# jsourati/nn-active-learning

Hardware: AMD Instinct MI355X
Metric: patches/sec Fisher-scored (32^3, 2-class) (higher is better)
Workload: dtype f32 (fp32 operands split into 16-bit pieces on the 16-bit MFMA, fp32 accumulate: fp16 pairs - 22-23 bits kept per operand, three products - in the conv under the head (forward + backward), in dec1's forward launch and in the other backward launches; bf16 triples - all 24 bits, exact, six products -

## Files before the change

### include/alq.h

```cpp
#ifndef ALQ_H
#define ALQ_H

#include <stddef.h>
#include <stdint.h>

#ifdef __cplusplus
extern "C" {
#endif

typedef struct alq_ctx alq_ctx;
typedef struct alq_model alq_model;

enum { ALQ_OK = 0, ALQ_EINVAL = -1, ALQ_EHIP = -2, ALQ_ENOMEM = -3, ALQ_EUNSUPPORTED = -4 };

enum { ALQ_CONV = 0, ALQ_CONVT = 1, ALQ_POOL = 2, ALQ_FC = 3 };

typedef struct {
    int32_t type;
    int32_t cout;
    int32_t k[3];
    int32_t s[3];
    int32_t relu;
    int32_t skip_src;
} alq_layer_t;
// ... 58 lines not shown

int alq_fisher_rows(alq_model *m, const float *d_pool, const int64_t *d_rows, int N, const float *d_p1_in,
                    double diag_load, float *d_p1_out, double *d_g0, double *d_g1, double *d_A,
                    double *d_trace, double *d_Asum);

int64_t alq_model_num_params(const alq_model *m);

int alq_forward_dropout(alq_model *m, const float *d_x, int N, float keep_prob, uint64_t seed, int64_t first_sample,
                        const int32_t *h_drop_layers, int n_drop_layers, float *d_post, int64_t *d_pred);

int alq_param_grads(alq_model *m, const float *d_x, int N, int mode, int cls, const int32_t *d_labels,
                    float loss_scale, float keep_prob, uint64_t seed, int64_t first_sample,
                    const int32_t *h_drop_layers, int n_drop_layers, int per_sample, float *d_grads,
                    float *d_post, double *d_loss);

int alq_grad_sqnorms(alq_model *m, const float *d_x, int N, int cls, const int32_t *d_cls,
                     float *d_post, double *d_sq);

int alq_hess_vecp(alq_model *m, const float *d_x, int N, const int32_t *d_labels, float loss_scale, const float *d_v,
                  const uint8_t *h_layer_on, int accumulate, double *d_hv, double *d_loss);

int alq_sgd_step(alq_ctx *ctx, float *d_theta, const float *d_grad, int64_t n, float lr);
int alq_adam_step(alq_ctx *ctx, float *d_theta, const float *d_grad, float *d_m, float *d_v, int64_t n, float lr,
                  float beta1, float beta2, float eps, int64_t t);
enum { ALQ_LOSS_CE = 0, ALQ_LOSS_CE_SOFT = 1, ALQ_LOSS_GCE = 2 };
typedef struct alq_loss_t {
    int32_t kind;
    float focal_gamma;
    float gce_q;
    float lwf_T;
    const float *d_class_w;
    const float *d_sample_w;
    const float *d_targets;
    const float *d_old_logits;
} alq_loss_t;

int alq_loss_stats(alq_ctx *ctx, const float *d_post, int c, int N, const int32_t *d_labels, const alq_loss_t *loss,
                   double *d_stats3);

int alq_param_grads_loss(alq_model *m, const float *d_x, int N, const int32_t *d_labels, const alq_loss_t *loss,
                         float loss_scale, float lwf_scale, float keep_prob, uint64_t seed, int64_t first_sample,
                         const int32_t *h_drop_layers, int n_drop_layers, float *d_grads, float *d_post, double *d_stats3);

int alq_rmsprop_step(alq_ctx *ctx, float *d_theta, const float *d_grad, float *d_ms, float *d_mom, int64_t n, float lr,
                     float decay, float momentum, float eps);

int alq_sq_accum(alq_ctx *ctx, const float *d_grads, int64_t per_sample_len, int N, double *d_acc);

int alq_shrink_sum(alq_ctx *ctx, const float *d_grads, int N, int64_t P, const int64_t *h_layer_elems, int L, double *d_out);
int alq_class_layer_sums(alq_model *m, const float *d_x, int N, int J, const int32_t *d_cls, float *d_post, double *d_g);

int alq_diag_fisher(alq_model *m, const float *d_x, int N, const int32_t *d_cls, double *d_acc);

size_t alq_topk_mask_work_bytes(int64_t n);
int alq_topk_mask(alq_ctx *ctx, const double *d_v, int64_t n, int64_t k, float *d_mask, void *d_work);
int alq_threshold_mask(alq_ctx *ctx, const double *d_v, int64_t n, double thr, float *d_mask);
int alq_fisher_classes(alq_ctx *ctx, const double *d_g, const double *d_w, const double *d_diag, int N, int c, int L,
                       double *d_A);

int alq_row_norms(alq_ctx *ctx, const float *d_A, int64_t n, int f, double *d_norms);
int alq_cosine_sims(alq_ctx *ctx, const float *d_A, int64_t n, const float *d_B, int b, int f, const double *d_na,
                    const double *d_nb, double *d_C);
size_t alq_colsum_work_bytes(int64_t n, int b);
int alq_colsum_max(alq_ctx *ctx, const double *d_S, int64_t n, int b, const double *d_cmax,
                   const unsigned char *d_skip, double *d_out, void *d_work);
int alq_take_colmax(alq_ctx *ctx, const double *d_S, int64_t n, int b, int j, int first, double *d_v);
int alq_fold_rowmax(alq_ctx *ctx, const double *d_S, int t, int64_t n, double *d_v);

int alq_local_var2d(alq_ctx *ctx, const void *d_vol, int vol_is_f64, const int64_t pad_dims[3], const int32_t rads[3], int d,
                    const int64_t *d_inds, int64_t n, double *d_out);
int alq_segment_min(alq_ctx *ctx, const int32_t *d_labels, const int64_t dims[3], int32_t n_labels, const int64_t *d_inds,
                    const double *d_scores, int64_t n, double *d_table);

size_t alq_cc_work_bytes(const int64_t dims[3]);
int alq_cc_label(alq_ctx *ctx, const uint8_t *d_seg, const int64_t dims[3], int connectivity, int select_zero, int32_t *d_labels);
int alq_cc_keep_largest(alq_ctx *ctx, const uint8_t *d_seg, const int64_t dims[3], int connectivity, int skip_origin, uint8_t *d_out,
                        int64_t *d_info, void *d_work);
int alq_fill_holes(alq_ctx *ctx, const uint8_t *d_seg, const int64_t dims[3], uint8_t *d_out, int64_t *d_info, void *d_work);

typedef struct alq_dcrf_params {
    float sdims_smooth[2];
    float sdims_app[2];
    float schan;
    float compat_smooth, compat_app;
    int32_t niter;
} alq_dcrf_params;
size_t alq_dcrf_work_bytes(const int64_t dims[3]);
int alq_dcrf2d(alq_ctx *ctx, const float *d_post, const float *d_img, const int64_t dims[3], const alq_dcrf_params *par,
               float *d_q1, uint8_t *d_map, void *d_work);

int alq_llfc_grads(alq_ctx *ctx, const float *d_feat, const float *d_post, const int32_t *d_labels, int n, int d, int c,
                   float *d_out);
size_t alq_llfc_hess_max_bytes(void);
int alq_llfc_hess(alq_ctx *ctx, const float *d_feat_one, const float *d_post_one, int d, int c, double *d_H);
int alq_llfc_if_path(int d, int c);
size_t alq_llfc_if_work_bytes(int n_pool, int c);
int alq_llfc_stoch_if(alq_ctx *ctx, const float *d_pool_feat, const float *d_pool_post, const int32_t *d_pool_labels, int n_pool,
                      const float *d_tr_feat, const float *d_tr_post, int n_tr, const int32_t *d_draws, int T, double scale, int d,
                      int c, int path, float *d_V, void *d_work);

int alq_aopt_tile(void);
int alq_aopt_max_workgroups(void);
size_t alq_aopt_work_bytes(int64_t n, int L);
int alq_aopt_svec(alq_ctx *ctx, const double *d_A, int64_t n, int L, double *d_V);
int alq_aopt_stats(alq_ctx *ctx, const double *d_V, const double *d_q, int64_t n, int m, const double *h_kvec,
                   const double *h_R, double mu, double obj, double *d_out, void *d_work);
int alq_aopt_direction(alq_ctx *ctx, const double *d_V, const double *d_q, int64_t n, int m, const double *h_kvec,
                       const double *h_R, const double *h_c_r, const double *h_c_1, double ratio, double mu, double obj,
                       double *d_dq, double *d_out, void *d_work);
int alq_aopt_linesearch(alq_ctx *ctx, const double *d_q, const double *d_dq, int64_t n, const double *h_alpha, int J,
                        double *d_out, void *d_work);
int alq_aopt_update(alq_ctx *ctx, double *d_q, const double *d_dq, const double *d_V, int64_t n, int m, double alpha,
                    double *d_out, void *d_work);

typedef struct {
    int32_t layer;
    int32_t pad;
    int64_t idx;
    double delta;
} alq_flip_t;
int alq_ref64_scores(alq_ctx *ctx, const alq_layer_t *layers, int n_layers, const int32_t in_dims[4],
                     const double *const *h_dW, const double *const *h_db, const float *d_x, const int64_t *d_rows, int N,
                     const alq_flip_t *d_flips, int flips_per_sample, double eps, int cand_cap,
                     double *d_logits, double *d_S, double *d_rms, alq_flip_t *d_cand, double *d_cand_key, int32_t *d_cand_count);

int alq_prof_enable(alq_ctx *ctx, int on);
int alq_prof_reset(alq_ctx *ctx);
int alq_prof_num_classes(void);
const char *alq_prof_class_name(int cls);
int alq_prof_read(alq_ctx *ctx, int cls, double *ms, int64_t *launches, double *flops);

int alq_model_debug_copy(alq_model *m, int layer_idx, int what, int N, float *d_out,
                         int64_t *elems_out);

int alq_debug_set_stamp_buffer(void *d_buf);
int alq_debug_set(int key, int value);
enum {
    ALQ_INFO_SUBNORMALS_OK = 0,
    ALQ_INFO_C3D_FWD = 1,
    ALQ_INFO_C3D_BWD = 2,
    ALQ_INFO_C3D_ONE_ACC = 3,
    ALQ_INFO_FLIP_OVERFLOW = 5,
    ALQ_INFO_F16_DERIVED = 6,
    ALQ_INFO_T3D_FWD = 7,
    ALQ_INFO_T3D_BWD = 8,
    ALQ_INFO_E3D_BWD = 9,
    ALQ_INFO_D3D_FWD = 10,
    ALQ_INFO_D3D_BWD = 11,
    ALQ_INFO_F3D_FWD = 12,
    ALQ_INFO_C3D_BWD_FORM = 13,
    ALQ_INFO_HOST_PACK_ELEMS = 14,
    ALQ_INFO_LSUM = 15,
    ALQ_INFO_DCP_FORM = 16,
    ALQ_INFO_E3D_BWD_FORM = 17
};
int alq_model_engine_info(alq_model *m, int what);

int alq_synth_patches(alq_ctx *ctx, uint64_t seed, int64_t first_id, int64_t n,
                      int64_t elems_per_patch, float *d_out);

#ifdef __cplusplus
}
#endif
#endif
```

### nn-active-learning_amd/csrc/alq_internal.h

```cpp
#pragma once
#include <hip/hip_runtime.h>

#include <cstdint>
#include <cstdio>
#include <memory>
#include <string>
#include <vector>

#include "alq.h"
#include "engine_switches.h"

namespace alq {

void set_error(const char *fmt, ...);

#define ALQ_HIP(expr)                                                                     \
    do {                                                                                  \
        hipError_t e_ = (expr);                                                           \
        if (e_ != hipSuccess) {                                                           \
            ::alq::set_error("%s:%d: %s -> %s", __FILE__, __LINE__, #expr,               \
                             hipGetErrorString(e_));                                      \
            return ALQ_EHIP;                                                              \
        }                                                                                 \
    } while (0)
// ... 244 lines not shown

struct Igemm4Args {
    const float *in;
    float *out;
    const void *W;
    const float *bias;
    const float *mask;
    float *osumA, *osumB;
    const int *tdesc;
    const int *sdesc;
    const int *pdesc;
    const int *ttab;
    const int *vdesc;
    int in_cs, in_c0, out_cs, out_c0, Co;
    int mask_cs, mask_c0, mask_from, mask_to, split;
    int N, PT, tpg, rows;
    int PX, PYX, PZ;
    int smz, smy, smx;
    int soz, soy, sox, OD, OH, OW;
    int MD, MH, MW;
    int nph, ngr, NP;
    int nslots, plane_bytes;
    int in_pstride, out_pstride, in_bytes;
    int relu, accumulate, pair, store_from;
    int cls_ok;
    int in_split_ch, in_delta, out_split, out_delta, mask_split, mask_delta;
    int tt_ints, pd_off, td_off, wbytes, abytes;
    int dbg_repeat;
    unsigned long long *dbg;
    const unsigned *src_bits;
    int bits_pstride, bits_bytes;
    const float *fc_W;
    float *fc_part;
    unsigned char *fc_bits;
    int fc_F;
    int f16_ein;
    int f16_ew;
    const unsigned *in_amax, *in_amax2;
    unsigned *out_amax;
    int amax_from;
    int wp;
    int src_presplit;
    int xcd_order;
    int zreuse;
    float flip_tau;
    int flip_cap;
    unsigned *flip_cnt;
    unsigned *flip_list;
    const unsigned char *mask_bits;
    unsigned char *sign_out;
};

struct G4Geom {
    int kind = 0;
    int cls[3] = {0, 0, 0};
    int ID = 1, IH = 1, IW = 1, Ci = 0;
    int OD = 1, OH = 1, OW = 1, Co = 0;
    int k[3] = {1, 1, 1}, s[3] = {1, 1, 1}, lo[3] = {0, 0, 0};
    bool flipped = false;
    double flops_per_patch = 0;
};

struct Igemm4Plan {
    bool ok = false;
    Igemm4Args a;
    int NTW = 1;
    int wp = 3;
    int xw = 0;
    std::shared_ptr<Igemm4Plan> alt16;
    bool multi = false;
    bool fic = false;
    int tune_fic = -1;
    int tune_epi = -1;
    size_t lds_bytes = 0;
    double flops_per_patch = 0;
    int Ci = 0, Co = 0;
    struct Unit { int chunk = 0, S = 0, w_off = 0; std::vector<int> tap; };
    std::vector<Unit> units;
    std::vector<int> h_tdesc, h_sdesc, h_pdesc, h_ttab, h_vdesc;
    int *d_tdesc = nullptr, *d_sdesc = nullptr, *d_pdesc = nullptr, *d_ttab = nullptr, *d_vdesc = nullptr;
    std::vector<unsigned short> h_W;
    void *d_W = nullptr;
    std::vector<unsigned short> h_W16;
    void *d_W16 = nullptr;
    int w16_exp = 0;
};
int igemm4_build_plan(const G4Geom &g, int max_batch, Igemm4Plan *plan, int wp = 3);
void igemm4_pack_weights(Igemm4Plan *plan, const std::vector<float> &Bmat );
int igemm4_launch(alq_ctx *ctx, const Igemm4Plan &plan, const View &in, const View &out, const float *bias,
                  int relu, int accumulate, int N, int prof_cls, const Igemm2Fuse *fuse);

struct C3dPlan {
    bool ok = false;
    int D = 0;
    int w_exp = 0;
    int oneacc = 1;
    double flops_per_patch = 0;
    std::vector<unsigned short> h_W;
    void *d_W = nullptr;
    std::vector<unsigned short> h_W7;
    void *d_W7 = nullptr;
};
void c3d_bwd7_pack(C3dPlan *plan, const std::vector<float> &Bmat);
int c3d_subnormals_ok(alq_ctx *ctx);
int c3d_fwd_build(const View &in, const View &out, const int k[3], const int lo[3], const int s[3], C3dPlan *plan);
void c3d_fwd_pack(C3dPlan *plan, const std::vector<float> &Bmat );
int c3d_fwd_launch(alq_ctx *ctx, const C3dPlan &plan, const View &in, const float *bias, int N, const unsigned *amaxA, const unsigned *amaxB,
                   const float *fc_W, float *fc_part, float *asum_part, unsigned char *fc_bits, float flip_tau);
int c3d_bwd_build(const View &fwd_in, const View &fwd_out, const int k[3], const int lo[3], const int s[3], C3dPlan *plan);
void c3d_bwd_pack(C3dPlan *plan, const std::vector<float> &Bmat_fwd );
void c3d_presplit_vec(const float *v, long long F, int e, std::vector<unsigned short> *out);
int c3d_bwd_launch(alq_ctx *ctx, const C3dPlan &plan, int N, const unsigned char *bits, const void *vec16, int e_in, const unsigned char *maskA,
                   float *dB, float *sumA, float *sumB, int rows_per_wave = 8);

struct T3dPlan {
    bool ok = false;
    int kind = 0;
    int w_exp = 0;
    double flops_per_patch = 0;
    std::vector<unsigned short> h_W;
    void *d_W = nullptr;
};
int t3d_build(const View &in, const View &out, const int k[3], const int lo[3], const int s[3], T3dPlan *fwd, T3dPlan *bwd);
void t3d_fwd_pack(T3dPlan *plan, const float *W );
void t3d_bwd_pack(T3dPlan *plan, const float *W);
void t3d8_fwd_pack(T3dPlan *plan, const float *W );
void t3d8_bwd_pack(T3dPlan *plan, const float *W );
int t3d8_bwd_launch(alq_ctx *ctx, const T3dPlan &plan, const View &dout, const View &din, int N, float in_bound, const unsigned char *mask_bits, float *dsum);
int t3d_fwd_launch(alq_ctx *ctx, const T3dPlan &plan, const View &in, const View &out, const float *bias, int N, float *osum, unsigned *out_amax);
int t3d_bwd_launch(alq_ctx *ctx, const T3dPlan &plan, const View &dout, const View &din, int N, float in_bound, const unsigned char *mask_bits,
                   float *dsum);

struct E3dPlan {
    bool ok = false;
    int w_exp = 0;
    double flops_per_patch = 0;
    std::vector<unsigned short> h_Whi, h_Wlo;
    void *d_Whi = nullptr, *d_Wlo = nullptr;
};
int e3d_build(const View &in, const View &out, const int k[3], const int lo[3], const int s[3], E3dPlan *plan);
void e3d_pack(E3dPlan *plan, const float *W );
int e3d_bwd_launch(alq_ctx *ctx, const E3dPlan &plan, int N, const float *skip, const float *dpool, const unsigned char *am2, const unsigned char *sg2,
                   const unsigned char *am1, const unsigned char *sg1, float *dsum2, float *dsum1, float in_bound,
                   bool rows );

struct D3dPlan {
    bool ok = false;
    int w_exp = 0;
    double flops_per_patch = 0;
    std::vector<unsigned short> h_Whi, h_Wlo;
    void *d_Whi = nullptr, *d_Wlo = nullptr;
    std::vector<unsigned short> h_Bhi, h_Blo;
    void *d_Bhi = nullptr, *d_Blo = nullptr;
};
void d3d_bwd_pack(D3dPlan *plan, const float *W);
int d3d_bwd_launch(alq_ctx *ctx, const D3dPlan &plan, int N, const float *dout, float in_bound, float *dinA, float *dinB, float *sumB);
int d3d_build(const View &in, const View &out, const int k[3], const int lo[3], const int s[3], D3dPlan *plan);
void d3d_pack(D3dPlan *plan, const float *W );
int d3d_fwd_launch(alq_ctx *ctx, const D3dPlan &plan, int N, const float *inA, const float *inB, const unsigned *amaxA, const unsigned *amaxB,
                   const float *bias, int relu, float *out, unsigned char *sg, float *osum);

struct F3dPlan {
    bool ok = false;
    int w_exp = 0;
    double flops_per_patch = 0;
    std::vector<unsigned short> h_Whi, h_Wlo;
    void *d_Whi = nullptr, *d_Wlo = nullptr;
};
int f3d_build(const View &in, const View &out, const int k[3], const int lo[3], const int s[3], F3dPlan *plan);
void f3d_pack(F3dPlan *plan, const float *W );
int f3d_fwd_launch(alq_ctx *ctx, const F3dPlan &plan, int N, const float *in, const unsigned *amax, const float *bias, float *out, unsigned char *sg,
                   float *osum, float *pout, unsigned char *parg, float *posum);

struct DirectArgs {
    const float *in;
    float *out;
    const float *W;
    const float *bias;
    float *osum;
    int in_cs, in_c0, Ci, ID, IH, IW;
    int out_cs, out_c0, Co, OD, OH, OW;
    int MD, MH, MW;
    int PT, TZ, TY, TX, HZ, HY, HX, rows;
    int minz, miny, minx;
    int ntaps, tnx, tny, tnz;
    int tilesZ, tilesY, tilesX;
    int N, relu;
};

struct DirectPlan {
    DirectArgs a;
    bool ok = false;
    size_t lds_bytes = 0;
    double flops_per_patch = 0;
    float *d_W = nullptr;
};

int direct_build_plan(const IgemmPlan &p1, DirectPlan *dp);
int direct_launch(alq_ctx *ctx, const DirectPlan &dp, const View &in, const View &out, const float *bias, int relu,
                  int N, float *osum, int prof_cls);
int direct_conv_pool_launch(alq_ctx *ctx, const float *d_W, const View &in, const View &out, const View &pout,
                            const float *bias, int relu, uint8_t *argmax, float *osum, float *posum, int N,
                            double flops_per_patch, unsigned *amax = nullptr, unsigned char *sg = nullptr, unsigned char *psg = nullptr);

struct FcGemmPlan {
    bool ok = false;
    int K = 0, N = 0;
    std::vector<unsigned short> h_W;
    void *d_W = nullptr;
    std::vector<unsigned short> h_W16;
    void *d_W16 = nullptr;
    int w_exp = 0;
    int form = 0;
};
int fcgemm_build_plan(int K, int N, FcGemmPlan *plan);
void fcgemm_pack_weights(FcGemmPlan *plan, const std::vector<float> &Bmat );
void fcgemm_pack_weights_f16(FcGemmPlan *plan, const std::vector<float> &Bmat );
int fcgemm_launch(alq_ctx *ctx, const FcGemmPlan &plan, const View &in, const View &out, const float *bias, int relu,
                  int M, int prof_cls, float in_bound = 0.f, unsigned *row_amax = nullptr);

int wpack_stats(alq_ctx *ctx, const float *d_W, int Co, long long F, void *d_scal);
int wpack_permute(alq_ctx *ctx, const float *d_W, float *d_Wp, int Co, int D, int H, int Wd, int C);
int wpack_fc(alq_ctx *ctx, const float *d_Wp, long long ld, int K, int N, int kmajor, void *d_W3, void *d_W16, const void *d_scal);

struct Gemm {
    IgemmPlan p1;
    Igemm2Plan p2;
    Igemm3Plan p3;
    Igemm4Plan p4;
    FcGemmPlan pfc;
    bool pfc_f16 = false;
    bool p3_f16 = false;
    unsigned *fc_row_amax = nullptr;
    DirectPlan pd;
};

int k_pool_fwd(alq_ctx *, const View &in, const View &out, uint8_t *argmax, const int w[3],
               const int lo[3], int N, float *osum = nullptr, bool *fused = nullptr);
int k_pool_bwd_first(alq_ctx *, const View &dout, const View &pool_out, const uint8_t *argmax, const int w[3],
                     int ID, int IH, int IW, int N, float *dsum, int accumulate, int use_signs = 0);
int k_pool_bwd(alq_ctx *, const View &dout, const View &din, const uint8_t *argmax,
               const int w[3], const int lo[3], int N, int accumulate, const View *mask_act = nullptr,
               float *dsum = nullptr, bool *fused = nullptr, int store_din = 1, int use_signs = 0);
int k_chansum(alq_ctx *, const View &in, float *field, int N);
int k_mask_chansum(alq_ctx *, const View &dact, const View *act_or_null, float *field, int N);
int boxdot_slabs(long long vox);
int boxdot_conv_slabs(int D, int H, int W, const int k[3]);
int boxdot_convT_slabs(int ID, int IH, int IW, const int k[3], const int s[3]);
int k_boxdot_conv(alq_ctx *, const float *dsum, const float *asum, const float *asum2, int D, int H, int W,
                  const int k[3], const int lo[3], int N, double *Spart, int nslab_max);
int k_boxdot_convT(alq_ctx *, const float *dsum, const float *asum, const float *asum2, int ID, int IH, int IW,
                   const int k[3], const int s[3], const int lo[3], int N, double *Spart, int nslab_max);
int k_fc_small_fwd(alq_ctx *, const float *act, int64_t F, const float *Wp, int nout, int N,
                   float *partials, int nslices, unsigned *maskbits = nullptr);
int k_fc_small_dsum_bits(alq_ctx *, const unsigned *maskbits, const float *wv, int64_t F, int N, float *dsum);
int k_fc_small_finish(alq_ctx *, const float *partials, int nslices, const float *bias, int nout,
                      int relu, int N, float *out);
int k_fc_small_finish_diff(alq_ctx *, const float *partials, int nslices, const float *bias, int N, float *out);
int k_fc_small_bwd(alq_ctx *, const float *delta, int nout, const float *Wp, int64_t F, int N,
                   float *dact, const float *mask_act = nullptr, float *dsum = nullptr, int C = 0,
                   bool *fused = nullptr);
int k_rowsum_field(alq_ctx *, const float *field, int64_t len, int N, float *out);
struct FwdBoundsArgs { int nl; float L[16]; float B[16]; int src2[16]; int from_input = 0; };
int k_rowmax_abs(alq_ctx *, const float *x, int N, long long K, unsigned *out);
int k_fwd_bounds(alq_ctx *, const unsigned *amax0, int N, int stride, const FwdBoundsArgs &a, unsigned *bound_all);
int flip_segments(int N);
int flip_list_len(int N);
int k_flip_fix(alq_ctx *, unsigned *list, unsigned *cnt, int cap, int N, const float *inA, const float *inB, int CA, int CB,
               int D, int H, int W, int kz, int ky, int kx, int lz, int ly, int lx, const float *W32, const float *bias, int Co,
               unsigned char *bits, long long F, unsigned *overflow = nullptr);
int k_rowmax_u32(alq_ctx *, const unsigned *in, int len, int N, unsigned *out);
int k_softmax(alq_ctx *, const float *logits, int c, int N, float *post_cN, int64_t *pred);
int k_fill_unit_cotangent(alq_ctx *, float *dlogits, int N);
int k_fisher_finalize(alq_ctx *, const double *Spart, const int *nslab, int nslab_max, int max_batch, double *S,
                      int L, const double *sizes, const float *post_cN, const float *p1_branch, int N,
                      double diag_load, float *p1_out, double *g0, double *g1, double *A, double *trace,
                      double *Apart, int *nblocks_out);
int k_reduce_Asum(alq_ctx *, const double *Apart, int nblocks, int LL, double *Asum);
int fc_small_slices(int64_t F);

int k_dropout(alq_ctx *, const View &t, int N, long long first_sample, unsigned long long seed, int layer, float keep_prob);
int k_logit_cotangent(alq_ctx *, const float *post_cN, int c, int N, int mode, int cls, const int *labels, float scale,
                      float *dlogits);
int k_ce_loss(alq_ctx *, const float *post_cN, int c, int N, const int *labels, double *d_out);
long long wgrad_partial_floats(const View &U, const View &V, const int k[3]);
int k_wgrad(alq_ctx *, const View &U, const View &V, const int k[3], const int s[3], const int lo[3], int N, int sum_n,
            float *partial, float *d_out, long long out_stride);
int k_bgrad(alq_ctx *, const View &delta, int N, int sum_n, float *d_out, long long out_stride);
int k_fc_wgrad(alq_ctx *, const float *delta, const View &a, int nout, int N, int sum_n, float *d_out, long long out_stride);
int k_sgd(alq_ctx *, float *theta, const float *g, long long n, float lr);
int k_loss_cotangent(alq_ctx *, const float *post_cN, int c, int N, const int *labels, const alq_loss_t *loss, float loss_scale,
                     float lwf_scale, float *dlogits, double *d_stats3);
int k_rmsprop(alq_ctx *, float *theta, const float *g, float *ms, float *mom, long long n, float lr, float decay, float momentum,
              float eps);
int k_adam(alq_ctx *, float *theta, const float *g, float *m, float *v, long long n, float lr_t, float b1, float b2, float eps);
int k_sq_accum(alq_ctx *, const float *g, long long per, int N, double *acc);
int k_shrink_sum(alq_ctx *, const float *g, int N, long long P, const long long *off, int L, double *out);
int k_fisher_classes(alq_ctx *, const double *g, const double *w, const double *diag, int N, int c, int L, double *A);

long long gnorm_partials(const View &U, const View &V, const int k[3], const int s[3], const int lo[3]);
int k_gnorm_weight(alq_ctx *, const View &U, const View &V, const int k[3], const int s[3], const int lo[3], int N, double *part,
                   double *d_sq, int ld, int col);
int k_gnorm_bias(alq_ctx *, const View &delta, int N, double *d_sq, int ld, int col);
int k_gnorm_fc(alq_ctx *, const float *delta, int nout, const View &a, int N, double *d_sq, int ld, int col);

long long dfisher_weight_scratch(const View &U, const View &V, const int k[3], const int s[3], const int lo[3], int max_batch);
int k_dfisher_weight(alq_ctx *, const View &U, const View &V, const int k[3], const int s[3], const int lo[3], int N, double *scratch,
                     double *d_acc);
int k_dfisher_bias(alq_ctx *, const View &delta, int N, double *scratch , double *d_acc);
// ... 67 lines not shown
```

### nn-active-learning_amd/csrc/d3d.hip

```cpp
#include "f16_pair.h"
#include "sweep_common.h"

#include <algorithm>
#include <cmath>
#include <cstdlib>
#include <cstring>
#include <vector>

namespace alq {

struct D3Args {
    const float *inA, *inB;
    const unsigned *amaxA, *amaxB;
    const unsigned short *Whi;
    const unsigned short *Wlo;
    const float *bias;
    float *out;
    unsigned char *sg;
    float *osum;
    int e_w;
    int relu;
    int N;
};

constexpr int D3_KG = 18 * 16;
constexpr int D3_ROWB = 4 * D3_KG;
constexpr int D3_SLOT = 2 * D3_ROWB;
constexpr int D3_PLANE = 18 * D3_SLOT;
constexpr int D3_STRIP = 2 * D3_PLANE;

#ifndef D3_PIPE
#define D3_PIPE 2
#endif
#ifndef D3_START
#define D3_START 1
#endif

struct D3Row { f32x4 a, b; };

__global__ __launch_bounds__(256) __attribute__((amdgpu_waves_per_eu(1, 1))) void d3d_fwd_kernel(const D3Args a) {
    extern __shared__ __attribute__((aligned(16))) char d3lds[];
    const int lane = threadIdx.x & 63, wave = __builtin_amdgcn_readfirstlane((int)(threadIdx.x >> 6));
    char *strip = d3lds;
    for (int i = threadIdx.x; i < D3_STRIP / 16; i += 256) reinterpret_cast<i32x4 *>(strip)[i] = i32x4{0, 0, 0, 0};
    __syncthreads();
    const int n = lane & 15, kg = lane >> 4;
    f16x8 wh[27], wl[27];
#pragma unroll
    for (int c = 0; c < 27; ++c) {
        wh[c] = *reinterpret_cast<const f16x8 *>(a.Whi + ((size_t)c * 64 + lane) * 8);
        wl[c] = *reinterpret_cast<const f16x8 *>(a.Wlo + ((size_t)c * 64 + lane) * 8);
    }
#pragma unroll
    for (int c = 0; c < 27; ++c) asm volatile("" : "+a"(wh[c]), "+a"(wl[c]));
    f32x4 bias4 = *reinterpret_cast<const f32x4 *>(a.bias + 4 * kg);
    asm volatile("" : "+v"(bias4));
    const float relu_floor = a.relu ? 0.f : -__builtin_inff();

    typedef const unsigned __attribute__((address_space(4))) *cu32p;
    const cu32p amaxA_c = (cu32p)(unsigned long long)a.amaxA, amaxB_c = (cu32p)(unsigned long long)a.amaxB;
    auto patch_exp = [&](int p) __attribute__((always_inline)) {
        const unsigned fa = amaxA_c[p], fb = amaxB_c[p];
        return sw_patch_exp(fa > fb ? fa : fb);
    };

    const __amdgpu_buffer_rsrc_t ia_rsrc = sw_rsrc(a.inA, (unsigned long long)a.N * 4096 * 64);
    const __amdgpu_buffer_rsrc_t ib_rsrc = sw_rsrc(a.inB, (unsigned long long)a.N * 4096 * 64);
    const __amdgpu_buffer_rsrc_t o_rsrc = sw_rsrc(a.out, (unsigned long long)a.N * 4096 * 64);
    const __amdgpu_buffer_rsrc_t s_rsrc = sw_rsrc(a.sg, a.sg ? (unsigned long long)a.N * 4096 * 4 : 0ull);
    const __amdgpu_buffer_rsrc_t u_rsrc = sw_rsrc(a.osum, a.osum ? (unsigned long long)a.N * 4096 * 4 : 0ull);

    const int sx = lane >> 2, cq = lane & 3;
    char *const w_base = strip + (4 * wave + 1) * D3_SLOT + (cq >> 1) * D3_KG + (sx + 1) * 16 + (cq & 1) * 8;
    const unsigned ldA = (unsigned)lane * 16u;
    const char *const f_base = strip + 4 * wave * D3_SLOT + kg * D3_KG + n * 16;
    const unsigned e_out = (unsigned)n * 64u + (unsigned)kg * 16u, e_sg = (unsigned)n * 4u + (unsigned)kg;
    const unsigned e_sum = kg == 0 ? (unsigned)n * 4u : SW_OOB;

    SW_PATCH_ORDER(a.N);

    D3Row RA[4];
    auto fetch = [&](int q) __attribute__((always_inline)) {
        const unsigned row0 = ((unsigned)patch_of(q >> 4) * 16u + (unsigned)(q & 15)) * 16u + 4u * (unsigned)wave;
#pragma unroll
        for (int r = 0; r < 4; ++r) {
            RA[r].a = __builtin_bit_cast(f32x4, __builtin_amdgcn_raw_buffer_load_b128(ia_rsrc, (int)ldA, sw_s((row0 + r) * 1024u), 0));
            RA[r].b = __builtin_bit_cast(f32x4, __builtin_amdgcn_raw_buffer_load_b128(ib_rsrc, (int)ldA, sw_s((row0 + r) * 1024u), 0));
        }
    };
    auto stage_unit = [&](auto U, int img, float sc, float sc11) __attribute__((always_inline)) {
        constexpr int u = decltype(U)::value, r = u >> 1, h = u & 1;
        char *dst = w_base + img * D3_PLANE + r * D3_SLOT + h * 2 * D3_KG;
        const f32x4 g = h ? RA[r].b : RA[r].a;
        const f16x2 h01 = __builtin_convertvector(f32x2{g.x * sc, g.y * sc}, f16x2), h23 = __builtin_convertvector(f32x2{g.z * sc, g.w * sc}, f16x2);
        const f16x2 l01 = __builtin_convertvector(f32x2{__builtin_fmaf((float)h01.x, -2048.f, g.x * sc11), __builtin_fmaf((float)h01.y, -2048.f, g.y * sc11)}, f16x2);
        const f16x2 l23 = __builtin_convertvector(f32x2{__builtin_fmaf((float)h23.x, -2048.f, g.z * sc11), __builtin_fmaf((float)h23.y, -2048.f, g.w * sc11)}, f16x2);
        *reinterpret_cast<i32x2 *>(dst) = i32x2{__builtin_bit_cast(int, h01), __builtin_bit_cast(int, h23)};
        *reinterpret_cast<i32x2 *>(dst + D3_ROWB) = i32x2{__builtin_bit_cast(int, l01), __builtin_bit_cast(int, l23)};
    };

    f32x4 acc[3][4], acx[3][4];
#pragma unroll
    for (int st = 0; st < 3; ++st)
#pragma unroll
        for (int ry = 0; ry < 4; ++ry) { acc[st][ry] = f32x4{0.f, 0.f, 0.f, 0.f}; acx[st][ry] = f32x4{0.f, 0.f, 0.f, 0.f}; }
    f32x4 okeep[2];
    okeep[0] = okeep[1] = f32x4{0.f, 0.f, 0.f, 0.f};

    auto epi_row = [&](auto ST, auto RY, int p, int zo, bool tv, float inv) __attribute__((always_inline)) {
        constexpr int st = decltype(ST)::value, ry = decltype(RY)::value;
        const unsigned vrow = (unsigned)sw_s((((unsigned)p * 16u + (unsigned)(tv ? zo : 0)) * 16u + (unsigned)(4 * wave + ry)) * 16u);
        const f32x4 c = acc[st][ry], cx = acx[st][ry];
        if (!D3_START) { acc[st][ry] = f32x4{0.f, 0.f, 0.f, 0.f}; acx[st][ry] = f32x4{0.f, 0.f, 0.f, 0.f}; }
        const float v0 = __builtin_fmaxf(__builtin_fmaf(__builtin_fmaf(cx.x, 0x1p-11f, c.x), inv, bias4.x), relu_floor);
        const float v1 = __builtin_fmaxf(__builtin_fmaf(__builtin_fmaf(cx.y, 0x1p-11f, c.y), inv, bias4.y), relu_floor);
        const float v2 = __builtin_fmaxf(__builtin_fmaf(__builtin_fmaf(cx.z, 0x1p-11f, c.z), inv, bias4.z), relu_floor);
        const float v3 = __builtin_fmaxf(__builtin_fmaf(__builtin_fmaf(cx.w, 0x1p-11f, c.w), inv, bias4.w), relu_floor);
        const f32x4 o = f32x4{v0, v1, v2, v3};
        okeep[ry & 1] = o;
        __builtin_amdgcn_raw_buffer_store_b128(__builtin_bit_cast(i32x4, o), o_rsrc, (int)(tv ? e_out : SW_OOB), (int)(vrow * 64u), 0);
        ALQ_STORE_HOLD("v"(o));
        const unsigned bits = (v0 > 0.f ? 1u : 0u) | (v1 > 0.f ? 2u : 0u) | (v2 > 0.f ? 4u : 0u) | (v3 > 0.f ? 8u : 0u);
        __builtin_amdgcn_raw_buffer_store_b8((unsigned char)bits, s_rsrc, (int)(tv ? e_sg : SW_OOB), (int)(vrow * 4u), 0);
        float s_ = (v0 + v1) + (v2 + v3);
        s_ += __shfl_xor(s_, 16, 64);
        s_ += __shfl_xor(s_, 32, 64);
        __builtin_amdgcn_raw_buffer_store_b32(__builtin_bit_cast(int, s_), u_rsrc, (int)(tv ? e_sum : SW_OOB), (int)(vrow * 4u), 0);
    };

    auto step = [&](auto JJ, int i, int s) __attribute__((always_inline)) {
        constexpr int J = decltype(JJ)::value;
        constexpr int S0 = (J + 1) % 3, S1 = J, S2 = (J + 2) % 3;
        __builtin_amdgcn_sched_barrier(0);
        const int q = 16 * i + s;
        const int p = patch_of(i);
        const float inv = __builtin_ldexpf(1.f, -(patch_exp(p) + a.e_w));
        const int pn = patch_of((q + 1) >> 4);
        const int cen = patch_exp(pn);
        const bool nv = ((q + 1) >> 4) < npw;
        const float sc = nv ? __builtin_ldexpf(1.f, cen) : 0.f, sc11 = nv ? __builtin_ldexpf(1.f, cen + 11) : 0.f;
        const int img = q & 1;
        asm volatile("s_waitcnt lgkmcnt(0)\n\ts_barrier" ::: "memory");
        const char *fb = f_base + img * D3_PLANE;
        f16x8 Fh[2][3], Fl[2][3];
        auto frag = [&](auto R, f16x8 *fh, f16x8 *fl) __attribute__((always_inline)) {
            constexpr int r = decltype(R)::value;
#pragma unroll
            for (int dx = 0; dx < 3; ++dx) {
                fh[dx] = *reinterpret_cast<const f16x8 *>(fb + r * D3_SLOT + dx * 16);
                fl[dx] = *reinterpret_cast<const f16x8 *>(fb + r * D3_SLOT + dx * 16 + D3_ROWB);
            }
        };
        frag(IC<0>{}, Fh[0], Fl[0]);
        auto block = [&](auto R) __attribute__((always_inline)) {
            constexpr int r = decltype(R)::value;
            __builtin_amdgcn_sched_barrier(0);
            if constexpr (r + 1 < 6) frag(IC<r + 1>{}, Fh[(r + 1) % 2], Fl[(r + 1) % 2]);
            if constexpr (r == 0) epi_row(IC<S0>{}, IC<3>{}, p, s - 2, s >= 2, inv);
            if constexpr (r == 1) { stage_unit(IC<0>{}, img ^ 1, sc, sc11); stage_unit(IC<1>{}, img ^ 1, sc, sc11); stage_unit(IC<2>{}, img ^ 1, sc, sc11); stage_unit(IC<3>{}, img ^ 1, sc, sc11); }
// ... 101 lines not shown
        wl[c] = *reinterpret_cast<const f16x8 *>(a.Wlo + ((size_t)(cb * 15 + c) * 64 + lane) * 8);
    }
#pragma unroll
    for (int c = 0; c < 15; ++c) asm volatile("" : "+a"(wh[c]), "+a"(wl[c]));

    const __amdgpu_buffer_rsrc_t i_rsrc = sw_rsrc(a.dout, (unsigned long long)a.N * 4096 * 64);
    const __amdgpu_buffer_rsrc_t o_rsrc = sw_rsrc(cb ? a.dinB : a.dinA, (unsigned long long)a.N * 4096 * 64);
    const __amdgpu_buffer_rsrc_t u_rsrc = sw_rsrc(a.sumB, a.sumB ? (unsigned long long)a.N * 4096 * 4 : 0ull);

    const int sx = lane >> 2, cq = lane & 3;
    char *const w_base = strip + (4 * wave + 1) * DB_SLOT + (cq >> 1) * DB_KG + (sx + 1) * 16 + (cq & 1) * 8;
    const unsigned ldA = (unsigned)lane * 16u;
    const char *const f01 = strip + 8 * rg * DB_SLOT + (kg & 1) * DB_KG + (n + (kg >> 1)) * 16;
    const char *const f22 = strip + 8 * rg * DB_SLOT + (kg >> 1) * DB_SLOT + (kg & 1) * DB_KG + (n + 2) * 16;
    const unsigned e_out = (unsigned)n * 64u + (unsigned)kg * 16u;
    const unsigned e_sum = (kg == 0 && cb == 1) ? (unsigned)n * 4u : SW_OOB;

    SW_PATCH_ORDER(a.N);

    f32x4 RA[4];
    auto fetch = [&](int q) __attribute__((always_inline)) {
        const unsigned row0 = ((unsigned)patch_of(q >> 4) * 16u + (unsigned)(q & 15)) * 16u + 4u * (unsigned)wave;
#pragma unroll
        for (int r = 0; r < 4; ++r)
            RA[r] = __builtin_bit_cast(f32x4, __builtin_amdgcn_raw_buffer_load_b128(i_rsrc, (int)ldA, sw_s((row0 + r) * 1024u), 0));
    };
    auto stage_unit = [&](auto U, int img, float sc, float sc11) __attribute__((always_inline)) {
        constexpr int r = decltype(U)::value;
        char *dst = w_base + img * DB_PLANE + r * DB_SLOT;
        const f32x4 g = RA[r];
        const f16x2 h01 = __builtin_convertvector(f32x2{g.x * sc, g.y * sc}, f16x2), h23 = __builtin_convertvector(f32x2{g.z * sc, g.w * sc}, f16x2);
        const f16x2 l01 = __builtin_convertvector(f32x2{__builtin_fmaf((float)h01.x, -2048.f, g.x * sc11), __builtin_fmaf((float)h01.y, -2048.f, g.y * sc11)}, f16x2);
        const f16x2 l23 = __builtin_convertvector(f32x2{__builtin_fmaf((float)h23.x, -2048.f, g.z * sc11), __builtin_fmaf((float)h23.y, -2048.f, g.w * sc11)}, f16x2);
        *reinterpret_cast<i32x2 *>(dst) = i32x2{__builtin_bit_cast(int, h01), __builtin_bit_cast(int, h23)};
        *reinterpret_cast<i32x2 *>(dst + DB_ROWB) = i32x2{__builtin_bit_cast(int, l01), __builtin_bit_cast(int, l23)};
    };

    f32x4 acc[3][8], acx[3][8];
#pragma unroll
    for (int st = 0; st < 3; ++st)
#pragma unroll
        for (int ry = 0; ry < 8; ++ry) { acc[st][ry] = f32x4{0.f, 0.f, 0.f, 0.f}; acx[st][ry] = f32x4{0.f, 0.f, 0.f, 0.f}; }
    f32x4 okeep[2];
    okeep[0] = okeep[1] = f32x4{0.f, 0.f, 0.f, 0.f};

    auto epi_row = [&](auto ST, auto RY, int p, int zo, bool tv) __attribute__((always_inline)) {
        constexpr int st = decltype(ST)::value, ry = decltype(RY)::value;
        const unsigned vrow = (unsigned)sw_s((((unsigned)p * 16u + (unsigned)(tv ? zo : 0)) * 16u + (unsigned)(8 * rg + ry)) * 16u);
        const f32x4 c = acc[st][ry], cx = acx[st][ry];
        if (!D3_START) { acc[st][ry] = f32x4{0.f, 0.f, 0.f, 0.f}; acx[st][ry] = f32x4{0.f, 0.f, 0.f, 0.f}; }
        const float v0 = __builtin_fmaf(cx.x, 0x1p-11f, c.x) * a.inv, v1 = __builtin_fmaf(cx.y, 0x1p-11f, c.y) * a.inv;
        const float v2 = __builtin_fmaf(cx.z, 0x1p-11f, c.z) * a.inv, v3 = __builtin_fmaf(cx.w, 0x1p-11f, c.w) * a.inv;
        const f32x4 o = f32x4{v0, v1, v2, v3};
        okeep[ry & 1] = o;
        __builtin_amdgcn_raw_buffer_store_b128(__builtin_bit_cast(i32x4, o), o_rsrc, (int)(tv ? e_out : SW_OOB), (int)(vrow * 64u), 0);
        ALQ_STORE_HOLD("v"(o));
        float s_ = (v0 + v1) + (v2 + v3);
        s_ += __shfl_xor(s_, 16, 64);
        s_ += __shfl_xor(s_, 32, 64);
        __builtin_amdgcn_raw_buffer_store_b32(__builtin_bit_cast(int, s_), u_rsrc, (int)(tv ? e_sum : SW_OOB), (int)(vrow * 4u), 0);
    };

    auto step = [&](auto JJ, int i, int s) __attribute__((always_inline)) {
        constexpr int J = decltype(JJ)::value;
        constexpr int S0 = (J + 1) % 3, S1 = J, S2 = (J + 2) % 3;
        __builtin_amdgcn_sched_barrier(0);
        const int q = 16 * i + s;
        const int p = patch_of(i);
        const bool nv = ((q + 1) >> 4) < npw;
        const float sc = nv ? a.scale : 0.f, sc11 = nv ? a.scale11 : 0.f;
        const int img = q & 1;
        asm volatile("s_waitcnt lgkmcnt(0)\n\ts_barrier" ::: "memory");
        const char *fa = f01 + img * DB_PLANE, *fb = f22 + img * DB_PLANE;
        f16x8 Fh[2][2], Fl[2][2];
        auto frag = [&](auto R, f16x8 *fh, f16x8 *fl) __attribute__((always_inline)) {
            constexpr int r = decltype(R)::value;
            fh[0] = *reinterpret_cast<const f16x8 *>(fa + r * DB_SLOT);
            fl[0] = *reinterpret_cast<const f16x8 *>(fa + r * DB_SLOT + DB_ROWB);
            fh[1] = *reinterpret_cast<const f16x8 *>(fb + r * DB_SLOT);
            fl[1] = *reinterpret_cast<const f16x8 *>(fb + r * DB_SLOT + DB_ROWB);
        };
        frag(IC<0>{}, Fh[0], Fl[0]);
        auto mm = [&](auto ST, auto RY, auto KS, const f16x8 &xh, const f16x8 &xl) __attribute__((always_inline)) {
            constexpr int st = decltype(ST)::value, ry = decltype(RY)::value, ks = decltype(KS)::value;
            constexpr bool first = D3_START && ks == 0;
            const f32x4 zero = f32x4{0.f, 0.f, 0.f, 0.f};
            acx[st][ry] = __builtin_amdgcn_mfma_f32_16x16x32_f16(wl[ks], xh, first ? zero : acx[st][ry], 0, 0, 0);
            acc[st][ry] = __builtin_amdgcn_mfma_f32_16x16x32_f16(wh[ks], xh, first ? zero : acc[st][ry], 0, 0, 0);
            acx[st][ry] = __builtin_amdgcn_mfma_f32_16x16x32_f16(wh[ks], xl, acx[st][ry], 0, 0, 0);
        };
        auto block = [&](auto R) __attribute__((always_inline)) {
            constexpr int r = decltype(R)::value;
            __builtin_amdgcn_sched_barrier(0);
            if constexpr (r + 1 < 10) frag(IC<r + 1>{}, Fh[(r + 1) % 2], Fl[(r + 1) % 2]);
            if constexpr (r == 0) epi_row(IC<S0>{}, IC<7>{}, p, s - 2, s >= 2);
            if constexpr (r == 2) { stage_unit(IC<0>{}, img ^ 1, sc, sc11); stage_unit(IC<1>{}, img ^ 1, sc, sc11); }
            if constexpr (r == 3) { stage_unit(IC<2>{}, img ^ 1, sc, sc11); stage_unit(IC<3>{}, img ^ 1, sc, sc11); }
            if constexpr (r == 4) fetch(q + 2);
            if constexpr (r >= 3) epi_row(IC<S2>{}, IC<r - 3>{}, p, s - 1, s >= 1);
            const f16x8 ph = Fh[r % 2][0], pl = Fl[r % 2][0], qh = Fh[r % 2][1], ql = Fl[r % 2][1];
#define D3B_ALLDZ(RYV, PIV, XH, XL)                                                   \
            mm(IC<S0>{}, IC<RYV>{}, IC<0 * 5 + PIV>{}, XH, XL);                 \
            mm(IC<S1>{}, IC<RYV>{}, IC<1 * 5 + PIV>{}, XH, XL);                 \
            mm(IC<S2>{}, IC<RYV>{}, IC<2 * 5 + PIV>{}, XH, XL);
            if constexpr (r <= 7) { D3B_ALLDZ((r <= 7 ? r : 0), 0, ph, pl) }
            if constexpr (r >= 1 && r <= 8) { D3B_ALLDZ((r >= 1 && r <= 8 ? r - 1 : 0), 1, ph, pl) }
            if constexpr (r >= 2) { D3B_ALLDZ((r >= 2 ? r - 2 : 0), 2, ph, pl) }
            if constexpr (r <= 7) { D3B_ALLDZ((r <= 7 ? r : 0), 3, qh, ql) }
            if constexpr (r >= 2) { D3B_ALLDZ((r >= 2 ? r - 2 : 0), 4, qh, ql) }
#undef D3B_ALLDZ
#pragma unroll
            for (int m = 0; m < 9 * ((r == 0 || r == 9) ? 2 : ((r == 1 || r == 8) ? 3 : 5)); ++m) {
                __builtin_amdgcn_sched_group_barrier(0x008, 1, 0);
                __builtin_amdgcn_sched_group_barrier(SW_FILL_MASK, D3_PIPE, 0);
            }
        };
        block(IC<0>{}); block(IC<1>{}); block(IC<2>{}); block(IC<3>{}); block(IC<4>{});
        block(IC<5>{}); block(IC<6>{}); block(IC<7>{}); block(IC<8>{}); block(IC<9>{});
        __builtin_amdgcn_sched_barrier(0);
        const f32x4 k0 = okeep[0], k1 = okeep[1];
        asm volatile("" :: "v"(k0), "v"(k1));
    };

    if (npw > 0) {
        {
            fetch(0);
            stage_unit(IC<0>{}, 0, a.scale, a.scale11); stage_unit(IC<1>{}, 0, a.scale, a.scale11);
            stage_unit(IC<2>{}, 0, a.scale, a.scale11); stage_unit(IC<3>{}, 0, a.scale, a.scale11);
            __builtin_amdgcn_sched_barrier(0);
            fetch(1);
        }
        for (int i = 0; i < npw; ++i) {
            for (int k = 0; k < 5; ++k) {
                step(IC<0>{}, i, 3 * k);
                step(IC<1>{}, i, 3 * k + 1);
                step(IC<2>{}, i, 3 * k + 2);
            }
            step(IC<0>{}, i, 15);
            __builtin_amdgcn_sched_barrier(0);
            const int p = patch_of(i);
            epi_row(IC<2>{}, IC<7>{}, p, 14, true);
            epi_row(IC<0>{}, IC<0>{}, p, 15, true); epi_row(IC<0>{}, IC<1>{}, p, 15, true);
            epi_row(IC<0>{}, IC<2>{}, p, 15, true); epi_row(IC<0>{}, IC<3>{}, p, 15, true);
            epi_row(IC<0>{}, IC<4>{}, p, 15, true); epi_row(IC<0>{}, IC<5>{}, p, 15, true);
            epi_row(IC<0>{}, IC<6>{}, p, 15, true); epi_row(IC<0>{}, IC<7>{}, p, 15, true);
#pragma unroll
            for (int ry = 0; ry < 8; ++ry) { acc[0][ry] = f32x4{0.f, 0.f, 0.f, 0.f}; acx[0][ry] = f32x4{0.f, 0.f, 0.f, 0.f}; }
            __builtin_amdgcn_sched_barrier(0);
            asm volatile("s_nop 7" :: "v"(okeep[0]), "v"(okeep[1]) : "memory");
        }
    }
}

int d3d_build(const View &in, const View &out, const int k[3], const int lo[3], const int s[3], D3dPlan *plan) {
    plan->ok = false;
    if (getenv("ALQ_NO_D3D")) return ALQ_OK;
    if (!is_conv3_same(k, lo, s)) return ALQ_OK;
    if (!(in.D == 16 && in.H == 16 && in.W == 16 && out.D == 16 && out.H == 16 && out.W == 16 && in.C == 32 && in.split == 16 && in.cs == 16 && in.c0 == 0 &&
          out.C == 16 && out.cs == 16 && out.c0 == 0 && out.split == 0)) return ALQ_OK;
    plan->flops_per_patch = 2.0 * 27 * 32 * 16 * 4096.0;
    plan->ok = true;
    return ALQ_OK;
}

void d3d_pack(D3dPlan *plan, const float *W) {
    plan->w_exp = f16_pair_exp(W, (size_t)27 * 32 * 16);
    plan->h_Whi.assign((size_t)27 * 64 * 8, 0);
    plan->h_Wlo.assign((size_t)27 * 64 * 8, 0);
    for (int tap = 0; tap < 27; ++tap)
        for (int lane = 0; lane < 64; ++lane) {
            const int co = lane & 15, kg = lane >> 4;
            for (int c = 0; c < 8; ++c) {
                const float w = W[((size_t)tap * 32 + 8 * kg + c) * 16 + co];
                const size_t o = ((size_t)tap * 64 + lane) * 8 + c;
                f16_pair_split(w, plan->w_exp, 11, &plan->h_Whi[o], &plan->h_Wlo[o]);
            }
        }
}

void d3d_bwd_pack(D3dPlan *plan, const float *W) {
    plan->h_Bhi.assign((size_t)2 * 15 * 64 * 8, 0);
    plan->h_Blo.assign((size_t)2 * 15 * 64 * 8, 0);
    for (int cb = 0; cb < 2; ++cb)
        for (int dz = 0; dz < 3; ++dz)
            for (int pi = 0; pi < 5; ++pi)
                for (int lane = 0; lane < 64; ++lane) {
                    const int r = lane & 15, kg = lane >> 4, h = kg >> 1;
                    int dy, dx;
                    bool any = true;
                    if (pi < 3) { dy = pi; dx = h; } else if (pi == 3) { dy = h; dx = 2; } else { dy = 2; dx = 2; any = h == 0; }
                    for (int c = 0; c < 8; ++c) {
                        const int co = 8 * (kg & 1) + c, ci = 16 * cb + r;
                        const int tap = ((2 - dz) * 3 + (2 - dy)) * 3 + (2 - dx);
                        const float w = any ? W[((size_t)tap * 32 + ci) * 16 + co] : 0.f;
                        const size_t o = ((size_t)((cb * 3 + dz) * 5 + pi) * 64 + lane) * 8 + c;
                        f16_pair_split(w, plan->w_exp, 11, &plan->h_Bhi[o], &plan->h_Blo[o]);
                    }
                }
}

int d3d_bwd_launch(alq_ctx *ctx, const D3dPlan &plan, int N, const float *dout, float in_bound, float *dinA, float *dinB, float *sumB) {
    ALQ_REQUIRE(plan.ok && plan.d_Bhi && plan.d_Blo, ALQ_EINVAL, "d3d: backward weights not set");
    ALQ_REQUIRE(dout && dinA && dinB && in_bound > 0.f, ALQ_EINVAL, "d3d: missing argument");
    SWEEP_REQUIRE_PATCHES(N, "d3d");
    if (N <= 0) return ALQ_OK;
    const int e_in = f16_pair_exp(&in_bound, 1);
    D3BArgs a;
    a.dout = dout; a.Whi = reinterpret_cast<const unsigned short *>(plan.d_Bhi); a.Wlo = reinterpret_cast<const unsigned short *>(plan.d_Blo);
    a.dinA = dinA; a.dinB = dinB; a.sumB = sumB;
    a.scale = std::ldexp(1.f, e_in); a.scale11 = std::ldexp(1.f, e_in + 11); a.inv = std::ldexp(1.f, -(e_in + plan.w_exp)); a.N = N;
    ProfScope ps(ctx, PROF_IGEMM_F16, plan.flops_per_patch * N);
    return sweep_launch(ctx, d3d_bwd_kernel, sweep_grid(ctx, N, 1), 256, DB_STRIP, a);
}

int d3d_fwd_launch(alq_ctx *ctx, const D3dPlan &plan, int N, const float *inA, const float *inB, const unsigned *amaxA, const unsigned *amaxB,
                   const float *bias, int relu, float *out, unsigned char *sg, float *osum) {
    ALQ_REQUIRE(plan.ok && plan.d_Whi && plan.d_Wlo, ALQ_EINVAL, "d3d: weights not set");
    ALQ_REQUIRE(inA && inB && amaxA && amaxB && bias && out, ALQ_EINVAL, "d3d: missing argument");
    SWEEP_REQUIRE_PATCHES(N, "d3d");
    if (N <= 0) return ALQ_OK;
    D3Args a;
    a.inA = inA; a.inB = inB; a.amaxA = amaxA; a.amaxB = amaxB;
    a.Whi = reinterpret_cast<const unsigned short *>(plan.d_Whi); a.Wlo = reinterpret_cast<const unsigned short *>(plan.d_Wlo);
    a.bias = bias; a.out = out; a.sg = sg; a.osum = osum; a.e_w = plan.w_exp; a.relu = relu; a.N = N;
    ProfScope ps(ctx, PROF_IGEMM_F16, plan.flops_per_patch * N);
    return sweep_launch(ctx, d3d_fwd_kernel, sweep_grid(ctx, N, 1), 256, D3_STRIP, a);
}

}
```

### nn-active-learning_amd/csrc/engine_switches.h

```cpp
#ifndef ALQ_ENGINE_SWITCHES_H
#define ALQ_ENGINE_SWITCHES_H
#include <cstddef>
#include <cstdlib>

namespace alq {

enum Knob {
    KNOB_REPEAT = 0,
    KNOB_FLAGS = 1,
    KNOB_NO_BWD_FUSE = 2,
    KNOB_NO_FWD_FUSE = 3,
    KNOB_NO_V3 = 4,
    KNOB_NO_V4 = 5,
    KNOB_NO_POOL_FIRST = 6,
    KNOB_NO_CONV_POOL = 7,
    KNOB_DCP_NARROW = 8,
    KNOB_E3D_GRID_CAP = 9,
    ALQ_NKNOBS = 10
};

struct EngineSwitches {
    int knobs[ALQ_NKNOBS] = {0, 0, 0, 0, 0, 0, 0, 0, 0, 0};
    int disable_v2 = 0;
    int disable_v3 = 0;
    int disable_v4 = 0;
    int no_fcgemm = 0;
    int no_split = 0;
    int no_wide2d_rule = 0;
    int no_v3_f16 = 0;
    int no_v3_f16_fwd = 0;
    int no_co_split = 0;
    int no_co_split_f16 = 0;
    int no_class_tiles = 0;
    int no_fc_bits = 0;
    int no_fc_fuse = 0;
    int no_fc_f16 = 0;
    int no_fc_f16_fwd = 0;
    int f16_derived_mask = 0;
    int has_f16_derived_mask = 0;
    int no_f16x2 = 0;
    int no_xcd_order = 0;
    int no_fixed = 0;
    int no_bound16 = 0;
    int no_flipfix = 0;
    int no_presplit = 0;
    int no_signs = 0;
    int no_signs0 = 0;
    int f16_fwd_mask = -1;
    int no_f16_derived = 0;
    int no_light_kernels = 0;
    int no_c3d = 0;
    int c3_bwd_rows = 7;
    int no_e3d = 0;
    int e3d_rows = 0;
    int no_d3d = 0;
    int no_d3b = 0;
    int no_f3d = 0;
    int no_t3d = 0;
};

enum SwitchRule {
    SW_PRESENT,
    SW_FIRST_IS_1,
    SW_ATOI_EQ,
    SW_INT,
    SW_ROWS
};

struct SwitchRow {
    const char *env;
    size_t member;
    SwitchRule rule;
    int arg;
};

#define ALQ_SW(env, member, rule, arg) {env, offsetof(EngineSwitches, member), rule, arg}
inline const SwitchRow kSwitchTable[] = {
    ALQ_SW("ALQ_DEBUG_REPEAT", knobs[KNOB_REPEAT], SW_INT, 0),
    ALQ_SW("ALQ_DEBUG_FLAGS", knobs[KNOB_FLAGS], SW_INT, 0),
    ALQ_SW("ALQ_NO_BWD_FUSE", knobs[KNOB_NO_BWD_FUSE], SW_INT, 0),
    ALQ_SW("ALQ_NO_FWD_FUSE", knobs[KNOB_NO_FWD_FUSE], SW_INT, 0),
    ALQ_SW("ALQ_NO_V3", knobs[KNOB_NO_V3], SW_INT, 0),
    ALQ_SW("ALQ_NO_V4", knobs[KNOB_NO_V4], SW_INT, 0),
    ALQ_SW("ALQ_NO_POOL_FIRST", knobs[KNOB_NO_POOL_FIRST], SW_INT, 0),
    ALQ_SW("ALQ_NO_CONV_POOL", knobs[KNOB_NO_CONV_POOL], SW_INT, 0),
    ALQ_SW("ALQ_DCP_NARROW", knobs[KNOB_DCP_NARROW], SW_INT, 0),
    ALQ_SW("ALQ_E3D_GRID_CAP", knobs[KNOB_E3D_GRID_CAP], SW_INT, 0),
    ALQ_SW("ALQ_DISABLE_V2", disable_v2, SW_FIRST_IS_1, 0),
    ALQ_SW("ALQ_DISABLE_V3", disable_v3, SW_FIRST_IS_1, 0),
    ALQ_SW("ALQ_DISABLE_V4", disable_v4, SW_PRESENT, 0),
    ALQ_SW("ALQ_NO_FCGEMM", no_fcgemm, SW_PRESENT, 0),
    ALQ_SW("ALQ_NO_SPLIT", no_split, SW_PRESENT, 0),
    ALQ_SW("ALQ_NO_WIDE2D_RULE", no_wide2d_rule, SW_PRESENT, 0),
    ALQ_SW("ALQ_NO_V3_F16", no_v3_f16, SW_PRESENT, 0),
    ALQ_SW("ALQ_NO_V3_F16_FWD", no_v3_f16_fwd, SW_PRESENT, 0),
    ALQ_SW("ALQ_NO_CO_SPLIT", no_co_split, SW_PRESENT, 0),
    ALQ_SW("ALQ_NO_CO_SPLIT_F16", no_co_split_f16, SW_PRESENT, 0),
    ALQ_SW("ALQ_NO_CLASS_TILES", no_class_tiles, SW_PRESENT, 0),
    ALQ_SW("ALQ_NO_FC_BITS", no_fc_bits, SW_PRESENT, 0),
    ALQ_SW("ALQ_NO_FC_FUSE", no_fc_fuse, SW_PRESENT, 0),
    ALQ_SW("ALQ_NO_FC_F16", no_fc_f16, SW_PRESENT, 0),
    ALQ_SW("ALQ_NO_FC_F16_FWD", no_fc_f16_fwd, SW_PRESENT, 0),
    ALQ_SW("ALQ_F16_DERIVED_MASK", f16_derived_mask, SW_INT, 0),
    ALQ_SW("ALQ_F16_DERIVED_MASK", has_f16_derived_mask, SW_PRESENT, 0),
    ALQ_SW("ALQ_NO_F16X2", no_f16x2, SW_PRESENT, 0),
    ALQ_SW("ALQ_NO_XCD_ORDER", no_xcd_order, SW_PRESENT, 0),
    ALQ_SW("ALQ_NO_FIXED", no_fixed, SW_PRESENT, 0),
    ALQ_SW("ALQ_NO_BOUND16", no_bound16, SW_PRESENT, 0),
    ALQ_SW("ALQ_NO_FLIPFIX", no_flipfix, SW_PRESENT, 0),
    ALQ_SW("ALQ_NO_PRESPLIT", no_presplit, SW_PRESENT, 0),
    ALQ_SW("ALQ_NO_SIGNS", no_signs, SW_PRESENT, 0),
    ALQ_SW("ALQ_NO_SIGNS0", no_signs0, SW_PRESENT, 0),
    ALQ_SW("ALQ_F16_FWD_MASK", f16_fwd_mask, SW_INT, 0),
    ALQ_SW("ALQ_F16_DERIVED", no_f16_derived, SW_ATOI_EQ, 0),
    ALQ_SW("ALQ_NO_F16_DERIVED", no_f16_derived, SW_ATOI_EQ, 1),
    ALQ_SW("ALQ_NO_LIGHT_KERNELS", no_light_kernels, SW_PRESENT, 0),
    ALQ_SW("ALQ_NO_C3D", no_c3d, SW_PRESENT, 0),
    ALQ_SW("ALQ_C3D_BWD_ROWS", c3_bwd_rows, SW_ROWS, 0),
    ALQ_SW("ALQ_NO_E3D", no_e3d, SW_PRESENT, 0),
    ALQ_SW("ALQ_E3D_ROWS", e3d_rows, SW_ATOI_EQ, 1),
    ALQ_SW("ALQ_NO_D3D", no_d3d, SW_PRESENT, 0),
    ALQ_SW("ALQ_NO_D3D_BWD", no_d3b, SW_PRESENT, 0),
    ALQ_SW("ALQ_NO_F3D", no_f3d, SW_PRESENT, 0),
    ALQ_SW("ALQ_NO_T3D", no_t3d, SW_PRESENT, 0),
};
#undef ALQ_SW
inline const int kNumSwitchRows = (int)(sizeof(kSwitchTable) / sizeof(kSwitchTable[0]));

inline int &switch_member(EngineSwitches &sw, const SwitchRow &row) {
    return *reinterpret_cast<int *>(reinterpret_cast<char *>(&sw) + row.member);
}

inline EngineSwitches read_engine_switches() {
    EngineSwitches sw;
    for (const SwitchRow &row : kSwitchTable) {
        const char *v = std::getenv(row.env);
        int &dst = switch_member(sw, row);
        switch (row.rule) {
            case SW_PRESENT:    if (v) dst = 1; break;
            case SW_FIRST_IS_1: if (v && v[0] == '1') dst = 1; break;
            case SW_ATOI_EQ:    if (v && std::atoi(v) == row.arg) dst = 1; break;
            case SW_INT:        if (v) dst = std::atoi(v); break;
            case SW_ROWS:       dst = (v && std::atoi(v) == 4) ? 4 : ((v && std::atoi(v) == 8) ? 8 : 7); break;
        }
    }
    return sw;
}

}
#endif
```

### nn-active-learning_amd/csrc/igemm2.hip

```cpp
#include "alq_internal.h"

#include <algorithm>
#include <cmath>
#include <cstring>

namespace alq {

typedef float f32x4 __attribute__((ext_vector_type(4)));
typedef float f32x2 __attribute__((ext_vector_type(2)));

#ifdef ALQ_STAMPS
#define STAMP(var) asm volatile("s_memtime %0\n\ts_waitcnt lgkmcnt(0)" : "=s"(var)::"memory")
#define PHASE_END(idx)                         \
    do {                                       \
        unsigned long long t_now_;             \
        STAMP(t_now_);                         \
        ph[idx] += t_now_ - t_last;            \
        t_last = t_now_;                       \
    } while (0)
#else
#define PHASE_END(idx) do {} while (0)
#endif

constexpr int I2_CBP = 12;
// ... 331 lines not shown
                        mm(a1, b1);
                        __builtin_amdgcn_sched_barrier(0);
                    }
                }
            }
            PHASE_END(6);
        }
        have_pend = true;
        p_out = c_out; p_cls = c_cls; p_l = c_l; p_g = c_g;
        more = next_more;
    }
    if (have_pend) flush();
#ifdef ALQ_STAMPS
    PHASE_END(7);
    if (a.dbg && tid == 0)
        for (int i = 0; i < 8; ++i) a.dbg[blockIdx.x * 8 + i] = ph[i];
#endif
}

int igemm2_build_plan(const IgemmPlan &p1, Igemm2Plan *p2) {
    p2->ok = false;
    const IgemmArgs &a1 = p1.a;
    if (p1.smallc || p1.CB != 8 || a1.NB != 1 || p1.NTW > 3 || a1.ntaps > 27 || a1.Co % 4) return ALQ_OK;
    const int halo = a1.HZ * a1.HY * a1.HX;
    const int nhv = a1.PT * halo;
    if (nhv * 2 > 256 * I2_MAXSLOT) return ALQ_OK;
    if (a1.HZ > 255 || a1.HY > 255 || a1.HX > 255 || a1.PT > 127) return ALQ_OK;
    const size_t wchunk = (size_t)a1.ntaps * p1.NTW * 128 * 4;
    size_t wres_max = I2_WRES_MAX;
    if (const char *e = getenv("ALQ_WRES_KB")) wres_max = (size_t)atoi(e) * 1024;
    const bool wres = wchunk * a1.nchunks <= wres_max * p1.NTW;
    const size_t wbytes = wres ? wchunk * a1.nchunks : wchunk;
    const size_t lds = wbytes + (size_t)nhv * I2_CBP * 4;
    if (lds > 156 * 1024) return ALQ_OK;
    Igemm2Args &a = p2->a;
    std::memset(&a, 0, sizeof(a));
    a.Ci = a1.Ci; a.ID = a1.ID; a.IH = a1.IH; a.IW = a1.IW;
    a.Co = a1.Co; a.OD = a1.OD; a.OH = a1.OH; a.OW = a1.OW;
    a.MD = a1.MD; a.MH = a1.MH; a.MW = a1.MW;
    a.sm = a1.sm; a.so = a1.so; a.ooffz = a1.ooffz; a.ooffy = a1.ooffy; a.ooffx = a1.ooffx;
    a.PT = a1.PT; a.TZ = a1.TZ; a.TY = a1.TY; a.TX = a1.TX; a.HZ = a1.HZ; a.HY = a1.HY; a.HX = a1.HX;
    a.rows = a1.rows; a.minz = a1.minz; a.miny = a1.miny; a.minx = a1.minx;
    a.ntaps = a1.ntaps; a.nchunks = a1.nchunks;
    a.tilesZ = a1.tilesZ; a.tilesY = a1.tilesY; a.tilesX = a1.tilesX;
    {
        std::vector<int> off(a1.ntaps);
        for (int t = 0; t < a1.ntaps; ++t) off[t] = a1.tapoff[t] / 10 * I2_CBP;
        bool found = false;
        for (int nx = 1; nx <= a1.ntaps && !found; ++nx) {
            if (a1.ntaps % nx) continue;
            for (int ny = 1; nx * ny <= a1.ntaps && !found; ++ny) {
                if ((a1.ntaps / nx) % ny) continue;
                const int nz = a1.ntaps / (nx * ny);
                const int sx = nx > 1 ? off[1] - off[0] : 0;
                const int sy = ny > 1 ? off[nx] - off[0] : 0;
                const int sz = nz > 1 ? off[nx * ny] - off[0] : 0;
                bool okb = true;
                for (int t = 0; t < a1.ntaps && okb; ++t) {
                    const int ix = t % nx, iy = (t / nx) % ny, iz = t / (nx * ny);
                    okb = off[t] == off[0] + iz * sz + iy * sy + ix * sx;
                }
                if (okb) {
                    a.t0 = off[0]; a.tsx = sx; a.tsy = sy; a.tsz = sz; a.tnx = nx; a.tny = ny;
                    found = true;
                }
            }
        }
        if (!found) return ALQ_OK;
    }
    a.split = 1 << 30;
    {
        const int dimsI[3] = {a.ID, a.IH, a.IW}, dimsM[3] = {a.MD, a.MH, a.MW};
        const int T[3] = {a.TZ, a.TY, a.TX}, tiles[3] = {a.tilesZ, a.tilesY, a.tilesX};
        const int mins[3] = {a.minz, a.miny, a.minx}, H[3] = {a.HZ, a.HY, a.HX};
        auto cls_of = [&](int d, int t) { return (t == 0 ? 1 : 0) | (t == tiles[d] - 1 ? 2 : 0); };
        auto valid1 = [&](int d, int t, int h) {
            const int c = t * T[d] * a.sm + mins[d] + h;
            return c >= 0 && c < dimsI[d];
        };
        for (int d = 0; d < 3; ++d)
            for (int t = 1; t + 1 < tiles[d]; ++t)
                for (int h = 0; h < H[d]; ++h)
                    if (!valid1(d, t, h)) return ALQ_OK;
        a.tpg = a.tilesZ * a.tilesY * a.tilesX;
        a.in_pstride = a.PT * a.ID * a.IH * a.IW;
        a.out_pstride = a.PT * a.OD * a.OH * a.OW;
        p2->h_tdesc.assign((size_t)a.tpg * 8, 0);
        for (int tz = 0; tz < a.tilesZ; ++tz)
            for (int ty = 0; ty < a.tilesY; ++ty)
                for (int tx = 0; tx < a.tilesX; ++tx) {
                    int *td = &p2->h_tdesc[(((size_t)tz * a.tilesY + ty) * a.tilesX + tx) * 8];
                    const int mz0 = tz * a.TZ, my0 = ty * a.TY, mx0 = tx * a.TX;
                    const int z0 = mz0 * a.sm + a.minz, y0 = my0 * a.sm + a.miny, x0 = mx0 * a.sm + a.minx;
                    td[0] = (z0 * a.IH + y0) * a.IW + x0;
                    td[1] = ((mz0 * a.so + a.ooffz) * a.OH + my0 * a.so + a.ooffy) * a.OW + mx0 * a.so + a.ooffx;
                    const int cls = cls_of(0, tz) | (cls_of(1, ty) << 2) | (cls_of(2, tx) << 4);
                    const bool full = a.rows == 256 && mz0 + a.TZ <= a.MD && my0 + a.TY <= a.MH && mx0 + a.TX <= a.MW;
                    td[2] = cls | (full ? 256 : 0);
                    td[3] = mz0; td[4] = my0; td[5] = mx0;
                }
        (void)dimsM;
        auto rep = [&](int d, int c) { return (c & 1) ? 0 : ((c & 2) ? tiles[d] - 1 : (tiles[d] > 2 ? 1 : 0)); };
        p2->h_sdesc.assign((size_t)nhv * 4, 0);
        for (int pt = 0; pt < a.PT; ++pt)
            for (int hz = 0; hz < a.HZ; ++hz)
                for (int hy = 0; hy < a.HY; ++hy)
                    for (int hx = 0; hx < a.HX; ++hx) {
                        const int hv = ((pt * a.HZ + hz) * a.HY + hy) * a.HX + hx;
                        int *sd = &p2->h_sdesc[(size_t)hv * 4];
                        sd[0] = ((pt * a.ID + hz) * a.IH + hy) * a.IW + hx;
                        unsigned long long m = 0;
                        for (int c = 0; c < 64; ++c) {
                            const int cz = c & 3, cy = (c >> 2) & 3, cx = (c >> 4) & 3;
                            if (valid1(0, rep(0, cz), hz) && valid1(1, rep(1, cy), hy) && valid1(2, rep(2, cx), hx))
                                m |= 1ull << c;
                        }
                        sd[1] = (int)(unsigned)(m & 0xffffffffull);
                        sd[2] = (int)(unsigned)(m >> 32);
                        sd[3] = (pt << 24) | (hz << 16) | (hy << 8) | hx;
                    }
    }
    p2->NTW = p1.NTW;
    p2->wres = wres;
    p2->lds_bytes = lds;
    int max_wgs = 2;
    if (const char *e = getenv("ALQ_MAX_WGS")) max_wgs = atoi(e);
    p2->wgs_per_cu = std::max<int>(1, std::min<int>(max_wgs, (int)((160 * 1024) / (lds + 512))));
    p2->flops_per_patch = p1.flops_per_patch;
    p2->ok = true;
    return ALQ_OK;
}

void igemm2_pack_weights(Igemm2Plan *p2, const std::vector<float> &Bmat) {
    const Igemm2Args &a = p2->a;
    const int NTW = p2->NTW, Ci = a.Ci, Co = a.Co;
    p2->h_W.assign((size_t)a.nchunks * a.ntaps * NTW * 128, 0.f);
    for (int ch = 0; ch < a.nchunks; ++ch)
        for (int tp = 0; tp < a.ntaps; ++tp)
            for (int nt = 0; nt < NTW; ++nt)
                for (int lane = 0; lane < 64; ++lane)
                    for (int s = 0; s < 2; ++s) {
                        const int c = ch * 8 + 2 * (lane >> 4) + s;
                        const int co = nt * 16 + (lane & 15);
                        if (co < Co)
                            p2->h_W[((((size_t)ch * a.ntaps + tp) * NTW + nt) * 64 + lane) * 2 + s] =
                                Bmat[((size_t)tp * Ci + c) * Co + co];
                    }
}

unsigned long long *g_igemm2_dbg = nullptr;
int g_no_f16x2 = 0;
int g_no_xcd_order = 0;
int g_no_fixed = 0;
int g_dbg_knobs[ALQ_NKNOBS] = {0, 0, 0, 0, 0, 0, 0, 0, 0, 0};

template <int NTW, bool WRES, int GEO, bool SUMS>
static int launch2_s(alq_ctx *ctx, const Igemm2Plan &plan, const Igemm2Args &a, unsigned grid) {
    auto kfn = igemm2_kernel<NTW, WRES, GEO, SUMS>;
    if (plan.lds_bytes > 64 * 1024)
        ALQ_HIP(hipFuncSetAttribute(reinterpret_cast<const void *>(kfn), hipFuncAttributeMaxDynamicSharedMemorySize,
                                    (int)plan.lds_bytes));
    hipLaunchKernelGGL(kfn, dim3(grid), dim3(256), plan.lds_bytes, ctx->stream, a);
    ALQ_HIP(hipGetLastError());
    return ALQ_OK;
}

template <int NTW, bool WRES, int GEO>
static int launch2_t(alq_ctx *ctx, const Igemm2Plan &plan, const Igemm2Args &a, unsigned grid) {
    return (a.osumA || a.osumB) ? launch2_s<NTW, WRES, GEO, true>(ctx, plan, a, grid)
                                : launch2_s<NTW, WRES, GEO, false>(ctx, plan, a, grid);
}

int igemm2_launch(alq_ctx *ctx, const Igemm2Plan &plan, const View &in, const View &out, const float *bias, int relu,
                  int accumulate, int N, int prof_cls, const Igemm2Fuse *fuse) {
    Igemm2Args a = plan.a;
    ALQ_REQUIRE(in.C == a.Ci && in.D == a.ID && in.H == a.IH && in.W == a.IW, ALQ_EINVAL,
                "igemm2: input view does not match plan");
    ALQ_REQUIRE(out.C == a.Co && out.D == a.OD && out.H == a.OH && out.W == a.OW, ALQ_EINVAL,
                "igemm2: output view does not match plan");
    ALQ_REQUIRE(plan.d_W != nullptr, ALQ_EINVAL, "igemm2: weights not set");
    ALQ_REQUIRE((long long)N * in.vox() * in.cs < (1LL << 29) && (long long)N * out.vox() * out.cs < (1LL << 29),
                ALQ_EUNSUPPORTED, "igemm2: tensor exceeds the 32-bit byte-offset range (lower the batch)");
    ALQ_REQUIRE(in.cs % 4 == 0 && in.c0 % 4 == 0 && out.cs % 4 == 0 && out.c0 % 4 == 0, ALQ_EUNSUPPORTED,
                "igemm2: channel slice not 16-byte aligned");
    if (fuse) ALQ_REQUIRE(fuse->split % 4 == 0 && fuse->mask_cs % 4 == 0 && fuse->mask_c0 % 4 == 0 && fuse->mask_from % 4 == 0, ALQ_EUNSUPPORTED,
                          "igemm2: fused epilogue needs 4-channel aligned slices");
    a.in = in.p; a.in_cs = in.cs; a.in_c0 = in.c0;
    a.out = out.p; a.out_cs = out.cs; a.out_c0 = out.c0;
    a.W = plan.d_W; a.bias = bias; a.relu = relu; a.accumulate = accumulate; a.N = N;
    a.in_bytes = (int)((long long)N * in.vox() * in.cs * 4);
    a.dbg = nullptr;
    if (g_igemm2_dbg) {
        static int want = -2;
        if (want == -2) { const char *e = getenv("ALQ_STAMP_ONLY"); want = e ? atoi(e) : -1; }
        static int ordinal = 0;
        static unsigned long long *last = nullptr;
        if (last != g_igemm2_dbg) { last = g_igemm2_dbg; ordinal = 0; }
        if (want < 0 || ordinal == want) a.dbg = g_igemm2_dbg;
        ++ordinal;
    }
    a.dbg_repeat = g_dbg_knobs[KNOB_REPEAT];
    a.dbg_flags = g_dbg_knobs[KNOB_FLAGS];
    if (fuse) {
        a.mask = fuse->mask; a.mask_cs = fuse->mask_cs; a.mask_c0 = fuse->mask_c0; a.mask_from = fuse->mask_from;
        a.osumA = fuse->osumA; a.osumB = fuse->osumB;
        a.split = fuse->split > 0 ? fuse->split : (1 << 30);
    }
    const int pgroups = (N + a.PT - 1) / a.PT;
    const long long total = (long long)pgroups * a.tilesZ * a.tilesY * a.tilesX;
    const unsigned grid = (unsigned)std::min<long long>(total, 256LL * plan.wgs_per_cu);
    ProfScope ps(ctx, prof_cls, plan.flops_per_patch * N);
    int geo = 0;
    if (a.ntaps == 27 && a.tnx == 3 && a.tny == 3 && a.HY == 6 && a.HX == 18) {
        const int SX = I2_CBP, SY = 18 * I2_CBP, SZ = 6 * 18 * I2_CBP;
        if (a.t0 == 0 && a.tsx == SX && a.tsy == SY && a.tsz == SZ) geo = 1;
        if (a.t0 == 2 * (SX + SY + SZ) && a.tsx == -SX && a.tsy == -SY && a.tsz == -SZ) geo = 2;
    }
#define ALQ_L2(NT)                                                                                       \
    case NT:                                                                                             \
        if (geo == 1) return plan.wres ? launch2_t<NT, true, 1>(ctx, plan, a, grid) : launch2_t<NT, false, 1>(ctx, plan, a, grid); \
        if (geo == 2) return plan.wres ? launch2_t<NT, true, 2>(ctx, plan, a, grid) : launch2_t<NT, false, 2>(ctx, plan, a, grid); \
        return plan.wres ? launch2_t<NT, true, 0>(ctx, plan, a, grid) : launch2_t<NT, false, 0>(ctx, plan, a, grid)
    switch (plan.NTW) { ALQ_L2(1); ALQ_L2(2); ALQ_L2(3); }
#undef ALQ_L2
    set_error("igemm2: NTW=%d unsupported", plan.NTW);
    return ALQ_EUNSUPPORTED;
}

}
```

### nn-active-learning_amd/csrc/model.hip

```cpp
#include <algorithm>
#include <cmath>
#include <cstdarg>
#include <cstring>
#include <string>

#include "model_types.h"

namespace alq {

static thread_local char g_err[1024] = "";
void set_error(const char *fmt, ...) {
    va_list ap;
    va_start(ap, fmt);
    vsnprintf(g_err, sizeof(g_err), fmt, ap);
    va_end(ap);
}

int gather_normalize_impl(alq_ctx *, const void *const *, int, int, const int64_t[3], const int64_t[3],
                          const int64_t *, int64_t, const int32_t[3], const double *, int, int, void *);
int score_entropy_impl(alq_ctx *, const float *, int64_t, double *, float *);
int synth_impl(alq_ctx *, uint64_t, int64_t, int64_t, int64_t, float *);
int gather_rows_impl(alq_ctx *, const float *, const int64_t *, int64_t, int64_t, float *);
int debug_view_copy(alq_ctx *, const View &, int, float *);
int debug_f64_copy(alq_ctx *, const double *, long long, float *);
size_t topk_work_bytes_impl(int64_t n);
int topk_impl(alq_ctx *, const double *, int64_t, int64_t, int64_t *, void *);

static void same_pads(int in, int k, int s, int *out, int *lo) {
    *out = (in + s - 1) / s;
    int total = (*out - 1) * s + k - in;
    if (total < 0) total = 0;
    *lo = total / 2;
}

}

using namespace alq;

int alq_ctx::prof_begin(int cls, hipEvent_t *e0, hipEvent_t *e1) {
    ProfSlot &s = prof[cls];
    auto get = [&](hipEvent_t *ev) -> int {
        if (!s.pool.empty()) {
            *ev = s.pool.back();
            s.pool.pop_back();
            return ALQ_OK;
        }
        return hipEventCreate(ev) == hipSuccess ? ALQ_OK : ALQ_EHIP;
    };
    if (get(e0) != ALQ_OK || get(e1) != ALQ_OK) return ALQ_EHIP;
    return hipEventRecord(*e0, stream) == hipSuccess ? ALQ_OK : ALQ_EHIP;
}

void alq_ctx::prof_end(int cls, hipEvent_t e0, hipEvent_t e1, double flops) {
    ProfSlot &s = prof[cls];
    (void)hipEventRecord(e1, stream);
    s.pending.emplace_back(e0, e1);
    s.launches += 1;
    s.flops += flops;
}

int alq_ctx::prof_collect() {
    ALQ_HIP(hipStreamSynchronize(stream));
    for (int c = 0; c < PROF_NUM; ++c) {
        ProfSlot &s = prof[c];
        for (auto &pr : s.pending) {
            float ms = 0.f;
            ALQ_HIP(hipEventElapsedTime(&ms, pr.first, pr.second));
            s.ms += ms;
            s.pool.push_back(pr.first);
            s.pool.push_back(pr.second);
        }
        s.pending.clear();
    }
    return ALQ_OK;
}

static int g_knob_override[ALQ_NKNOBS] = {-1, -1, -1, -1, -1, -1, -1, -1, -1, -1};

static void apply_knobs(const alq_model *m) {
    for (int k = 0; k < ALQ_NKNOBS; ++k) g_dbg_knobs[k] = g_knob_override[k] >= 0 ? g_knob_override[k] : m->sw.knobs[k];
    g_no_f16x2 = m->sw.no_f16x2;
    g_no_xcd_order = m->sw.no_xcd_order;
    g_no_fixed = m->sw.no_fixed;
}

static int gemm_build(const EngineSwitches &sw, const ConvDesc &d, int max_batch, Gemm *g, const G4Geom *g4 = nullptr) {
    ALQ_TRY(igemm_build_plan(d, max_batch, &g->p1));
    if (g4 && !sw.disable_v4) {
        G4Geom gg = *g4;
        gg.flops_per_patch = g->p1.flops_per_patch;
        ALQ_TRY(igemm4_build_plan(gg, max_batch, &g->p4));
    }
    ALQ_TRY(igemm2_build_plan(g->p1, &g->p2));
    ALQ_TRY(direct_build_plan(g->p1, &g->pd));
    if (sw.disable_v2) { g->p2.ok = false; g->pd.ok = false; }
    ALQ_TRY(igemm3_build_plan(g->p2, &g->p3));
    if (d.ID == 1 && d.IH == 1 && d.IW == 1 && d.tz.size() == 1 && d.sm == 1 && d.so == 1 && !sw.no_fcgemm)
        ALQ_TRY(fcgemm_build_plan(d.Ci, d.Co, &g->pfc));
    if (sw.disable_v3) g->p3.ok = false;
    return ALQ_OK;
}

static int prepare_call(alq_model *m, bool fisher) {
    m->last.call_fisher = fisher;
    apply_knobs(m);
    if (!two_slot_allowed()) ALQ_TRY(refresh_fallback_forms(m));
    return ALQ_OK;
}

enum GemmRoute { ROUTE_DIRECT, ROUTE_FCGEMM, ROUTE_IGEMM4, ROUTE_IGEMM3, ROUTE_IGEMM2, ROUTE_IGEMM };
static GemmRoute gemm_route(const Gemm &g, const View &in, const View &out, int accumulate, const Igemm2Fuse *fuse) {
    if (g.pd.ok && !accumulate && !(fuse && (fuse->mask || fuse->osumB || fuse->split))) return ROUTE_DIRECT;
    if (g.pfc.ok && !accumulate && !fuse && two_slot_allowed()) return ROUTE_FCGEMM;
    const bool split_view = in.split != 0 || out.split != 0;
    if (g.p4.ok && (two_slot_allowed() || split_view)) return ROUTE_IGEMM4;
    if (g.p3.ok && !g_dbg_knobs[KNOB_NO_V3]) return ROUTE_IGEMM3;
    return g.p2.ok ? ROUTE_IGEMM2 : ROUTE_IGEMM;
}

static int gemm_launch(alq_ctx *ctx, const Gemm &g, const View &in, const View &out, const float *bias, int relu,
                       int accumulate, int N, int cls, const Igemm2Fuse *fuse = nullptr, bool *fused = nullptr, float fc_in_bound = 0.f) {
    const GemmRoute route = gemm_route(g, in, out, accumulate, fuse);
    ALQ_REQUIRE(route <= ROUTE_FCGEMM || g.p4.ok || (in.split == 0 && out.split == 0), ALQ_EUNSUPPORTED, "split concat view without a two-slot plan");
    if (fused) *fused = fuse != nullptr && route != ROUTE_FCGEMM && route != ROUTE_IGEMM;
    const int cls3 = cls == PROF_IGEMM_BWD ? PROF_IGEMM3_BWD : PROF_IGEMM3_FWD;
    switch (route) {
        case ROUTE_DIRECT: return direct_launch(ctx, g.pd, in, out, bias, relu, N, fuse ? fuse->osumA : nullptr, PROF_DIRECT);
        case ROUTE_FCGEMM:
            return fcgemm_launch(ctx, g.pfc, in, out, bias, relu, N, cls3, (g_no_f16x2 || bias || relu) ? 0.f : fc_in_bound,
                                 (cls == PROF_IGEMM_FWD && !g_no_f16x2) ? g.fc_row_amax : nullptr);
        case ROUTE_IGEMM4: return igemm4_launch(ctx, g.p4, in, out, bias, relu, accumulate, N, cls3, fuse);
        case ROUTE_IGEMM3: return igemm3_launch(ctx, g.p2, g.p3, in, out, bias, relu, accumulate, N, cls3, fuse);
        case ROUTE_IGEMM2: return igemm2_launch(ctx, g.p2, in, out, bias, relu, accumulate, N, cls, fuse);
        case ROUTE_IGEMM: break;
    }
    return igemm_launch(ctx, g.p1, in, out, bias, relu, accumulate, N, cls);
}

static void enum_taps(const int k[3], std::vector<int> *tz, std::vector<int> *ty, std::vector<int> *tx) {
    for (int z = 0; z < k[0]; ++z)
        for (int y = 0; y < k[1]; ++y)
            for (int x = 0; x < k[2]; ++x) {
                tz->push_back(z); ty->push_back(y); tx->push_back(x);
            }
}

static int build_model(alq_model *m, const alq_layer_t *specs, int n_layers) {
    const EngineSwitches &sw = m->sw;
    m->layers.resize(n_layers);
    struct Shp { int D, H, W, C; };
    std::vector<Shp> outs(n_layers);
    Shp cur = {m->in_dims[0], m->in_dims[1], m->in_dims[2], m->in_dims[3]};
    bool flat = false;
    int pidx = 0;
    std::vector<int> src_of(n_layers, -1);
    std::vector<int> dest_of(n_layers, -1);
    for (int i = 0; i < n_layers; ++i) {
        Layer &ly = m->layers[i];
        ly.spec = specs[i];
        const alq_layer_t &sp = ly.spec;
        Shp in = cur;
        if (sp.skip_src >= 0) {
            ALQ_REQUIRE(sp.skip_src < i - 1, ALQ_EUNSUPPORTED, "layer %d: skip source %d must be an earlier, non-adjacent layer", i, sp.skip_src);
            ALQ_REQUIRE(dest_of[sp.skip_src] < 0, ALQ_EUNSUPPORTED, "layer %d feeds more than one concat", sp.skip_src);
            const Shp &s = outs[sp.skip_src];
            ALQ_REQUIRE(!flat && s.D == cur.D && s.H == cur.H && s.W == cur.W, ALQ_EUNSUPPORTED,
                        "layer %d: concat of maps of different size (resize_image_with_crop_or_pad) is outside the scored path", i);
            in.C = cur.C + s.C;
            src_of[i] = sp.skip_src;
            dest_of[sp.skip_src] = i;
        }
        Shp o = in;
        switch (sp.type) {
            case ALQ_CONV: {
                ALQ_REQUIRE(!flat, ALQ_EINVAL, "layer %d: conv after fc", i);
                ALQ_REQUIRE(sp.s[0] == 1 && sp.s[1] == 1 && sp.s[2] == 1, ALQ_EUNSUPPORTED, "layer %d: strided conv", i);
                for (int d = 0; d < 3; ++d) {
                    int od;
                    same_pads((&in.D)[d], sp.k[d], 1, &od, &ly.lo[d]);
                }
                o.C = sp.cout;
                ly.pidx = pidx++;
                ly.w_elems = (int64_t)sp.k[0] * sp.k[1] * sp.k[2] * in.C * sp.cout;
                ly.b_elems = sp.cout;
                break;
            }
            case ALQ_CONVT: {
                ALQ_REQUIRE(!flat, ALQ_EINVAL, "layer %d: conv_transpose after fc", i);
                for (int d = 0; d < 3; ++d) {
                    ALQ_REQUIRE(sp.k[d] >= sp.s[d], ALQ_EUNSUPPORTED, "layer %d: conv_transpose kernel < stride", i);
                    int od;
                    same_pads((&in.D)[d] * sp.s[d], sp.k[d], sp.s[d], &od, &ly.lo[d]);
                }
                ALQ_REQUIRE(sp.s[0] == sp.s[1] || in.D == 1, ALQ_EUNSUPPORTED, "layer %d: anisotropic stride", i);
                ALQ_REQUIRE(sp.s[1] == sp.s[2], ALQ_EUNSUPPORTED, "layer %d: anisotropic stride", i);
                o.D = in.D * sp.s[0]; o.H = in.H * sp.s[1]; o.W = in.W * sp.s[2];
                o.C = sp.cout;
                ly.pidx = pidx++;
                ly.w_elems = (int64_t)sp.k[0] * sp.k[1] * sp.k[2] * in.C * sp.cout;
                ly.b_elems = sp.cout;
                break;
            }
            case ALQ_POOL: {
                ALQ_REQUIRE(!flat, ALQ_EINVAL, "layer %d: pool after fc", i);
                for (int d = 0; d < 3; ++d) {
                    ALQ_REQUIRE(sp.k[d] == sp.s[d], ALQ_EUNSUPPORTED, "layer %d: pool window != stride", i);
                    ALQ_REQUIRE(sp.k[0] * sp.k[1] * sp.k[2] <= 255, ALQ_EUNSUPPORTED, "layer %d: pool window too large", i);
                    same_pads((&in.D)[d], sp.k[d], sp.s[d], &(&o.D)[d], &ly.lo[d]);
                }
                break;
            }
            case ALQ_FC: {
                ly.F = (int64_t)in.D * in.H * in.W * in.C;
                o = {1, 1, 1, sp.cout};
                ly.pidx = pidx++;
                ly.w_elems = ly.F * sp.cout;
                ly.b_elems = sp.cout;
                flat = true;
                break;
            }
            default:
                ALQ_REQUIRE(false, ALQ_EINVAL, "layer %d: unknown type %d", i, sp.type);
        }
        outs[i] = o;
        cur = o;
    }
    m->L = pidx;
    ALQ_REQUIRE(n_layers > 0 && specs[n_layers - 1].type == ALQ_FC, ALQ_EUNSUPPORTED,
                "the scored path needs an fc head (get_gradients, NN_extended.py:1025)");
    m->nclass = outs[n_layers - 1].C;
// ... 588 lines not shown
                        fu = &hz;
                    }
                    bool f2 = false;
                    ALQ_TRY(gemm_launch(ctx, ly.fwd[0], in, ly.out, ly.d_bias, ly.spec.relu, 0, N, PROF_IGEMM_FWD, fu, &f2));
                    fused = fuse ? f2 : false;
                }
                ly.signs_ready = sg_here;
                if (fuse && prod[i]) ALQ_TRY(k_rowmax_u32(ctx, m->amax_tiles, ly.fwd[0].p4.a.tpg * 4, N, ly.amax_fwd));
                break;
            }
            case ALQ_CONVT: {
                if (t3d_fwd_applies(m, i, prod, cons, with_sums, drop)) {
                    const bool want_amax = prod[i] != 0;
                    ALQ_TRY(t3d_fwd_launch(ctx, ly.t3f, in, ly.out, ly.d_bias, N, with_sums ? ly.osum : nullptr, want_amax ? m->amax_tiles : nullptr));
                    if (want_amax) ALQ_TRY(k_rowmax_u32(ctx, m->amax_tiles, 16, N, ly.amax_fwd));
                    ly.signs_ready = false;
                    fused = true;
                    m->last.fwd.t3f += 1;
                    break;
                }
                if (ly.fwd_all.ok && two_slot_allowed()) {
                    const bool want_amax = fuse && prod[i];
                    if (fuse) take_amax(fz, i);
                    if (want_amax) fz.out_amax = m->amax_tiles;
                    const bool sg_here = with_sums && fuse && !m->sw.no_signs && ly.spec.relu && ly.out.sg;
                    if (sg_here) fz.sign_out = ly.out.sg;
                    ALQ_TRY(igemm4_launch(ctx, ly.fwd_all, in, ly.out, ly.d_bias, ly.spec.relu, 0, N, PROF_IGEMM3_FWD, fuse));
                    ly.signs_ready = sg_here;
                    if (want_amax)
                        ALQ_TRY(k_rowmax_u32(ctx, m->amax_tiles, ly.fwd_all.a.tpg * (ly.fwd_all.multi ? ly.fwd_all.a.ngr : 1) * 4, N, ly.amax_fwd));
                    fused = fuse != nullptr;
                    break;
                }
                bool all = true;
                for (auto &p : ly.fwd) {
                    bool f1 = false;
                    ALQ_TRY(gemm_launch(ctx, p, in, ly.out, ly.d_bias, ly.spec.relu, 0, N, PROF_IGEMM_FWD, fuse, &f1));
                    all = all && f1;
                }
                fused = all;
                break;
            }
            case ALQ_POOL:
                ALQ_TRY(k_pool_fwd(ctx, in, ly.out, ly.argmax, ly.spec.k, ly.lo, N, with_sums ? ly.osum : nullptr, &fused));
                break;
            case ALQ_FC:
                if (with_sums) {
                    const bool prev_spatial = i > 0 && m->layers[i - 1].osum != nullptr;
                    if (c3_head) ALQ_TRY(k_rowsum_field(ctx, ly.c3_asum, 4, N, ly.asum));
                    else if (prev_spatial) ALQ_TRY(k_rowsum_field(ctx, m->layers[i - 1].osum, m->layers[i - 1].out.vox(), N, ly.asum));
                    else ALQ_TRY(k_chansum(ctx, flat_view(in), ly.asum, N));
                }
                if (ly.dense_fc_small && fc_head_fused) {
                    ALQ_TRY(k_fc_small_finish_diff(ctx, c3_head ? ly.c3_part : ly.fc_part2, c3_head ? 4 : ly.fc_slices2, ly.d_bias, N, ly.out.p));
                } else if (ly.dense_fc_small) {
                    ALQ_TRY(k_fc_small_fwd(ctx, in.p, ly.F, ly.d_Wp, ly.spec.cout, N, ly.fc_partials, ly.fc_slices,
                                           with_sums ? ly.fc_maskbits : nullptr));
                    ALQ_TRY(k_fc_small_finish(ctx, ly.fc_partials, ly.fc_slices, ly.d_bias, ly.spec.cout,
                                              ly.spec.relu, N, ly.out.p));
                } else {
                    ALQ_TRY(gemm_launch(ctx, ly.fwd[0], flat_view(in), ly.out, ly.d_bias, ly.spec.relu, 0, N,
                                        PROF_IGEMM_FWD));
                }
                break;
        }
        if (drop && drop->on(i)) {
            ALQ_REQUIRE(keep_all && !with_sums, ALQ_EINVAL, "dropout only in passes that keep every activation");
            ALQ_TRY(k_dropout(ctx, ly.spec.type == ALQ_FC ? flat_view(ly.out) : ly.out, N, drop->first_sample, drop->seed, i, drop->keep_prob));
        }
        if (with_sums && ly.osum && !fused) ALQ_TRY(k_chansum(ctx, ly.out, ly.osum, N));
        if (with_sums && i == 0 && ly.pidx == 0 && ly.spec.type != ALQ_FC && in.C > 1)
            ALQ_TRY(k_chansum(ctx, in, ly.asum, N));
    }
    return ALQ_OK;
}

struct SideStream {
    alq_ctx *c;
    hipStream_t main;
    bool on = false;
    explicit SideStream(alq_ctx *ctx) : c(ctx), main(ctx->stream) {
        if (!c->side || c->side_off) return;
        if (hipEventRecord(c->ev_fork, main) != hipSuccess || hipStreamWaitEvent(c->side, c->ev_fork, 0) != hipSuccess) {
            (void)hipGetLastError();
            return;
        }
        c->stream = c->side;
        c->side_used = true;
        on = true;
    }
    ~SideStream() { if (on) c->stream = main; }
    SideStream(const SideStream &) = delete;
    SideStream &operator=(const SideStream &) = delete;
};

static int side_join(alq_ctx *c) {
    if (!c->side || !c->side_used) return ALQ_OK;
    c->side_used = false;
    ALQ_HIP(hipEventRecord(c->ev_join, c->side));
    ALQ_HIP(hipStreamWaitEvent(c->stream, c->ev_join, 0));
    return ALQ_OK;
}


static bool pool_first_ok(const Layer &pl, const Layer &src) {
    return pl.spec.type == ALQ_POOL && src.pidx == 0 && src.spec.type != ALQ_FC && pl.spec.k[1] == 2 && pl.spec.k[2] == 2 &&
           (pl.spec.k[0] == 1 || pl.spec.k[0] == 2) && pl.lo[0] == 0 && pl.lo[1] == 0 && pl.lo[2] == 0 &&
           src.out.D == pl.out.D * pl.spec.k[0] && src.out.H == pl.out.H * 2 && src.out.W == pl.out.W * 2 &&
           (pl.out.C == 4 || pl.out.C == 8 || pl.out.C == 16) && ((pl.dout.cs | pl.dout.c0 | pl.out.cs | pl.out.c0) & 3) == 0 &&
           src.spec.relu && !g_dbg_knobs[KNOB_NO_POOL_FIRST];
}

static bool e3d_bwd_applies(const alq_model *m, int i, bool prev_is_src) {
    const Layer &ly = m->layers[i];
    if (!(ly.spec.type == ALQ_POOL && i >= 3 && !m->sw.no_e3d && two_slot_allowed() && !g_no_f16x2 && !m->sw.no_bound16 && !m->sw.no_signs &&
          !g_dbg_knobs[KNOB_NO_BWD_FUSE] && !g_dbg_knobs[KNOB_NO_POOL_FIRST]))
        return false;
    const Layer &cv = m->layers[i - 1], &p1 = m->layers[i - 2], &c0 = m->layers[i - 3];
    return cv.spec.type == ALQ_CONV && cv.e3b.ok && cv.e3b.d_Whi && cv.spec.relu && cv.signs_ready && cv.out.sg && prev_is_src &&
           p1.spec.type == ALQ_POOL && pool_first_ok(p1, c0) && c0.dsum_partial && p1.signs_ready && p1.out.sg && p1.spec.k[0] == 2 &&
           ly.spec.k[0] == 2 && ly.spec.k[1] == 2 && ly.spec.k[2] == 2 && ly.lo[0] == 0 && ly.lo[1] == 0 && ly.lo[2] == 0 &&
           ly.dout.D == 8 && ly.dout.H == 8 && ly.dout.W == 8 && ly.dout.C == 16 && ly.dout.cs == 16 && ly.dout.c0 == 0 && !ly.dout.split &&
           cv.dout.cs == 16 && cv.dout.c0 == 0 && !cv.dout.split && cv.out.cs == 16 && cv.out.c0 == 0 && p1.out.cs == 8 && p1.out.c0 == 0 &&
           p1.out.C == 8 && c0.out.D == 32 && cv.dout_bound > 0.f && cv.dsum && c0.dsum;
}

static bool head_bits_apply(const alq_model *m, int i, bool prev_param, bool prev_is_src) {
    const Layer &ly = m->layers[i];
    const Layer *prev = i > 0 ? &m->layers[i - 1] : nullptr;
    return ly.dense_fc_small && ly.fc_maskbits && prev_param && prev->out.cs == prev->out.C &&
           prev->out.c0 == 0 && two_slot_allowed() && prev->bwd.p4.ok && prev->bwd.p4.NTW == 1 && !prev->bwd.p4.multi &&
           prev->bwd.p4.a.PT == 1 && !prev->dout.split && !prev_is_src &&
           !(i >= 2 && m->layers[i - 2].out_is_skip_src && prev->spec.skip_src < 0);
}

static bool c3d_bwd_applies(const alq_model *m, const Layer &ly, const unsigned short *vec16c, const Igemm2Fuse *fuse, int acc) {
    return ly.c3b.ok && ly.c3b.d_W && vec16c && !m->sw.no_c3d && !g_no_f16x2 && fuse && !acc && fuse->in_vec_amax > 0.f &&
           fuse->split == 8 && fuse->store_from == 8 && fuse->mask_bits && fuse->mask_from == 0 && fuse->mask_to == 8 && fuse->osumA && fuse->osumB &&
           ly.din.split == 8 && ly.din.cs == 8 && ly.din.C == 16;
}

static bool t3d_bwd_applies(const alq_model *m, const Layer &ly, const Igemm2Fuse *fuse, int acc, bool hand, bool prev_param) {
    return ly.spec.type == ALQ_CONVT && ly.t3b.ok && ly.t3b.d_W && !m->sw.no_t3d && two_slot_allowed() && !g_no_f16x2 && !acc && fuse && !hand &&
           fuse->in_bound > 0.f && !fuse->in_amax && fuse->split == 0 && fuse->store_from == 0 && fuse->osumA && !fuse->osumB && fuse->mask_from == 0 &&
           (!fuse->mask || fuse->mask_bits) && !ly.dout.split && !ly.din.split && prev_param;
}

static bool d3d_bwd_applies(const alq_model *m, const Layer &ly, const Igemm2Fuse *fuse, int acc, bool hand) {
    return ly.spec.type == ALQ_CONV && ly.d3f.ok && ly.d3f.d_Bhi && !m->sw.no_d3d && !m->sw.no_d3b && two_slot_allowed() && !g_no_f16x2 && !acc && fuse && !hand &&
           fuse->in_bound > 0.f && !fuse->in_amax && fuse->split == 16 && fuse->store_from == 0 && !fuse->mask && !fuse->osumA && fuse->osumB &&
           !ly.dout.split && ly.dout.cs == 16 && ly.dout.c0 == 0 && ly.din.split == 16 && ly.din.cs == 16 && ly.din.c0 == 0 && ly.din.C == 32;
}

static int run_backward_main(alq_model *m, const float *d_x, int N);
static int run_backward(alq_model *m, const float *d_x, int N) {
    const int rc = run_backward_main(m, d_x, N);
    const int rj = side_join(m->ctx);
    return rc != ALQ_OK ? rc : rj;
}

static int run_backward_main(alq_model *m, const float *d_x, int N) {
    alq_ctx *ctx = m->ctx;
    const int nl = (int)m->layers.size();
    ALQ_REQUIRE(m->nclass == 2, ALQ_EUNSUPPORTED, "Fisher scoring is binary (PW_NNAL.py:766), got %d classes", m->nclass);
    ALQ_TRY(k_fill_unit_cotangent(ctx, m->dlogits, N));
    for (Layer &l : m->layers) { l.delta_ready = false; l.dsum_partial = false; l.dout_bits = nullptr; l.dout_vec = nullptr; l.dout_vec16 = nullptr; l.dout_vec16c = nullptr; l.dout_amax = nullptr; }
    m->last.bwd = {};
    {
        for (Layer &l : m->layers) l.dout_bound = 0.f;
        m->layers[nl - 1].dout_bound = 1.f;
        for (int i = nl - 1; i >= 1; --i) {
            const Layer &ly = m->layers[i];
            double inb = ly.dout_bound;
            if (ly.spec.type == ALQ_FC)
                inb = (ly.spec.cout == 2 && ly.fc_wv_amax > 0.f && i == nl - 1) ? (double)ly.fc_wv_amax : (i < nl - 1 ? ly.bwd_l1 * ly.dout_bound : 0.0);
            else if (ly.spec.type != ALQ_POOL) inb = ly.bwd_l1 * ly.dout_bound;
            if (!(inb > 0.0) || ly.dout_bound <= 0.f) inb = 0.0;
            auto add = [&](Layer &p) { p.dout_bound = (p.dout_bound < 0.f || inb <= 0.0) ? -1.f : p.dout_bound + (float)(inb * (1.0 + 1e-6)); };
            add(m->layers[i - 1]);
            if (ly.spec.skip_src >= 0) add(m->layers[ly.spec.skip_src]);
        }
    }
    int e3_conv = -1;
    for (int i = nl - 1; i >= 0; --i) {
        Layer &ly = m->layers[i];
        const bool prev_is_src = (i > 0 && m->layers[i - 1].out_is_skip_src && ly.spec.skip_src < 0);
        if (e3d_bwd_applies(m, i, prev_is_src)) {
            Layer &cv = m->layers[i - 1], &p1 = m->layers[i - 2], &c0 = m->layers[i - 3];
            ALQ_TRY(e3d_bwd_launch(ctx, cv.e3b, N, cv.dout.p, ly.dout.p, ly.argmax, cv.out.sg, p1.argmax, p1.out.sg, cv.dsum, c0.dsum, cv.dout_bound, m->sw.e3d_rows != 0));
            m->last.bwd.e3b_form = m->sw.e3d_rows ? 1 : 2;
            cv.delta_ready = true;
            c0.delta_ready = true;
            e3_conv = i - 1;
            m->last.bwd.e3b = 1;
            continue;
        }
        if (e3_conv >= 0 && i == e3_conv - 1) continue;
        Layer *prev = i > 0 ? &m->layers[i - 1] : nullptr;
        const bool prev_param = prev && prev->pidx >= 0 && prev->spec.type != ALQ_FC;
        if (ly.spec.type == ALQ_POOL && prev_param && pool_first_ok(ly, *prev) && (prev->dsum_partial || !prev_is_src)) {
            ALQ_TRY(k_pool_bwd_first(ctx, ly.dout, ly.out, ly.argmax, ly.spec.k, prev->out.D, prev->out.H, prev->out.W, N,
                                     prev->dsum, prev->dsum_partial ? 1 : 0, ly.signs_ready ? 1 : 0));
            prev->delta_ready = true;
            continue;
        }
        if (ly.spec.type == ALQ_POOL) {
            bool fused = false;
            ALQ_TRY(k_pool_bwd(ctx, ly.dout, ly.din, ly.argmax, ly.spec.k, ly.lo, N, prev_is_src ? 1 : 0,
                               (prev_param && prev->spec.relu) ? &prev->out : nullptr, prev_param ? prev->dsum : nullptr,
                               &fused, !(prev_param && prev->pidx == 0),
                               (prev_param && prev->signs_ready) ? 1 : 0));
            if (prev_param && fused) prev->delta_ready = true;
            continue;
        }
        const bool isfc = ly.spec.type == ALQ_FC;
        if (!ly.delta_ready) {
            View dv = isfc ? flat_view(ly.dout) : ly.dout;
            View av = isfc ? flat_view(ly.out) : ly.out;
            ALQ_TRY(k_mask_chansum(ctx, dv, ly.spec.relu ? &av : nullptr, ly.dsum, N));
        }
        const float *as1 = ly.asum, *as2 = nullptr;
        if (!isfc) {
            if (i == 0) as1 = ly.in.C == 1 ? d_x : ly.asum;
            else as1 = m->layers[i - 1].osum;
            if (ly.spec.skip_src >= 0) as2 = m->layers[ly.spec.skip_src].osum;
        }
        double *Sdst = m->Spart + (size_t)ly.pidx * m->max_batch * m->nslab_max;
        {
            SideStream beside(ctx);
            if (ly.spec.type == ALQ_CONVT) {
                ALQ_TRY(k_boxdot_convT(ctx, ly.dsum, as1, as2, ly.in.D, ly.in.H, ly.in.W, ly.spec.k, ly.spec.s, ly.lo, N, Sdst, m->nslab_max));
            } else if (isfc) {
                const int one[3] = {1, 1, 1}, zero[3] = {0, 0, 0};
                ALQ_TRY(k_boxdot_conv(ctx, ly.dsum, ly.asum, nullptr, 1, 1, 1, one, zero, N, Sdst, m->nslab_max));
            } else {
                ALQ_TRY(k_boxdot_conv(ctx, ly.dsum, as1, as2, ly.out.D, ly.out.H, ly.out.W, ly.spec.k, ly.lo, N, Sdst, m->nslab_max));
            }
        }
        if (ly.pidx == 0) break;
        if (i == e3_conv) continue;
        const int acc = prev_is_src ? 1 : 0;
        bool fused = false;
        if (isfc) {
            ALQ_REQUIRE(!acc, ALQ_EUNSUPPORTED, "layer %d: fc consumer of a skip source", i);
            if (head_bits_apply(m, i, prev_param, prev_is_src)) {
                {
                    SideStream beside(ctx);
                    ALQ_TRY(k_fc_small_dsum_bits(ctx, ly.fc_maskbits, ly.fc_wv, ly.F, N, prev->dsum));
                }
                prev->dout_bits = ly.fc_maskbits;
                prev->dout_vec = ly.fc_wv;
                prev->dout_vec16 = ly.fc_wv16;
                prev->dout_vec16c = ly.fc_wv16c;
                prev->dout_vec_amax = ly.spec.cout == 2 ? ly.fc_wv_amax : 0.f;
                fused = true;
            } else if (ly.dense_fc_small) {
                const bool can = prev_param && prev->out.cs == prev->out.C;
                ALQ_TRY(k_fc_small_bwd(ctx, ly.dout.p, ly.spec.cout, ly.d_Wp, ly.F, N, ly.din.p,
                                       (can && prev->spec.relu) ? prev->out.p : nullptr, can ? prev->dsum : nullptr,
                                       can ? prev->out.C : 0, &fused));
            } else {
                ALQ_TRY(gemm_launch(ctx, ly.bwd, ly.dout, flat_view(ly.din), nullptr, 0, 0, N, PROF_IGEMM_BWD, nullptr, nullptr,
                                    (ly.dout_bound > 0.f && !m->sw.no_bound16) ? ly.dout_bound : 0.f));
            }
        } else {
            Igemm2Fuse fz;
            const Igemm2Fuse *fuse = nullptr;
            if (prev_param && !g_dbg_knobs[KNOB_NO_BWD_FUSE]) {
                const int Cs = ly.spec.skip_src >= 0 ? m->layers[ly.spec.skip_src].out.C : 0;
                if (prev->spec.relu) {
                    fz.mask = prev->out.p; fz.mask_cs = prev->out.cs; fz.mask_c0 = prev->out.c0; fz.mask_from = Cs;
                    if (prev->signs_ready) fz.mask_bits = prev->out.sg;
                }
                if (Cs > 0) { fz.split = Cs; fz.osumB = prev->dsum; } else { fz.osumA = prev->dsum; }
                if (Cs > 0 && (two_slot_allowed() || ly.din.split) && ly.bwd.p4.ok) {
                    Layer &sl = m->layers[ly.spec.skip_src];
                    const bool next_pool = ly.spec.skip_src + 1 < nl && pool_first_ok(m->layers[ly.spec.skip_src + 1], sl);
                    const bool sliced = sl.out.p == prev->out.p && sl.out.cs == prev->out.cs && prev->out.c0 == sl.out.c0 + Cs;
                    const bool splitv = ly.in.split == Cs && sl.out.p == ly.in.p;
                    if (next_pool && (sliced || splitv) && (Cs & 3) == 0) {
                        fz.mask = sl.out.p; fz.mask_cs = sl.out.cs; fz.mask_c0 = sl.out.c0; fz.mask_from = 0;
                        fz.mask_bits = (sl.signs_ready && (!prev->spec.relu || prev->signs_ready)) ? sl.out.sg : nullptr;
                        if (splitv) { fz.mask_split = Cs; fz.mask_delta = ly.in.delta; }
                        if (!prev->spec.relu) fz.mask_to = Cs;
                        fz.osumA = sl.dsum; fz.store_from = Cs;
                        sl.dsum_partial = true;
                    }
                }
                fuse = &fz;
            }
            if (ly.dout_bits) {
                fz.in_bits = ly.dout_bits; fz.in_vec = ly.dout_vec; fz.in_vec_amax = ly.dout_vec_amax;
                fz.in_vec16 = m->sw.no_presplit ? nullptr : ly.dout_vec16;
                const unsigned short *vec16c = ly.dout_vec16c;
                ly.dout_bits = nullptr; ly.dout_vec = nullptr; ly.dout_vec16 = nullptr; ly.dout_vec16c = nullptr;
                const bool honoured = fuse != nullptr;
                const bool c3 = c3d_bwd_applies(m, ly, vec16c, fuse, acc);
                m->last.bwd.c3_bwd = c3;
                if (c3) {
                    int ex = 0;
                    (void)std::frexp(fz.in_vec_amax, &ex);
                    ALQ_TRY(c3d_bwd_launch(ctx, ly.c3b, N, reinterpret_cast<const unsigned char *>(fz.in_bits), vec16c, 14 - ex, fz.mask_bits,
                                           ly.din.p + ly.din.delta, fz.osumA, fz.osumB, m->sw.c3_bwd_rows));
                } else {
                    ALQ_TRY(igemm4_launch(ctx, ly.bwd.p4, ly.dout, ly.din, nullptr, 0, acc, N, PROF_IGEMM3_BWD, &fz));
                }
                fused = honoured;
            } else {
                const bool p4_here = fuse && two_slot_allowed() && ly.bwd.p4.ok && !ly.bwd.p4.multi && ly.bwd.p4.a.PT == 1 && !g_no_f16x2;
                bool hand = false;
                if (p4_here && prev_param && !acc && !(prev->dout_bound > 0.f && !m->sw.no_bound16) && prev->pidx > 0 && prev->bwd.p4.ok && !prev->bwd.p4.multi && prev->bwd.p4.a.PT == 1 &&
                    prev->bwd.p4.d_W16 && !prev->dout.split &&
                    ((prev->bwd.p4.NTW == 1 && prev->bwd.p4.fic) || prev->bwd.p4.NTW == 2)) {
                    const size_t len = (size_t)ly.bwd.p4.a.tpg * 4;
                    if (!m->amax_a) { ALQ_TRY(m->dalloc(&m->amax_a, (size_t)m->max_batch)); ALQ_TRY(m->dalloc(&m->amax_b, (size_t)m->max_batch)); }
                    ALQ_TRY(ensure_amax_tiles(m, len));
                    fz.out_amax = m->amax_tiles;
                    fz.amax_from = fz.split > 0 && fz.split < (1 << 29) ? fz.split : 0;
                    hand = true;
                }
                if (p4_here && !acc && ly.dout_amax) fz.in_amax = ly.dout_amax;
                if (p4_here && !acc && !fz.in_amax && ly.dout_bound > 0.f && !m->sw.no_bound16) fz.in_bound = ly.dout_bound;
                if (!fuse && !acc && two_slot_allowed() && ly.bwd.p4.ok && !ly.bwd.p4.multi && ly.bwd.p4.a.PT == 1 && !g_no_f16x2 && !ly.dout_amax &&
                    ly.dout_bound > 0.f && !m->sw.no_bound16 && !g_dbg_knobs[KNOB_NO_BWD_FUSE]) {
                    fz = Igemm2Fuse();
                    fz.in_bound = ly.dout_bound;
                    fuse = &fz;
                }
                if (!ly.bwd.p4.ok && ly.bwd.p3.ok && ly.bwd.p3.d_W16 && !acc && !g_no_f16x2 && ly.dout_bound > 0.f && !m->sw.no_bound16 && !g_dbg_knobs[KNOB_NO_BWD_FUSE] &&
                    two_slot_allowed() && !ly.bwd.pd.ok && !ly.bwd.pfc.ok) {
                    if (!fuse) { fz = Igemm2Fuse(); fuse = &fz; }
                    fz.in_bound = ly.dout_bound;
                }
                const unsigned *mine = ly.dout_amax;
                ly.dout_amax = nullptr;
                if (t3d_bwd_applies(m, ly, fuse, acc, hand, prev_param)) {
                    ALQ_TRY(t3d_bwd_launch(ctx, ly.t3b, ly.dout, ly.din, N, fz.in_bound, fz.mask ? fz.mask_bits : nullptr, fz.osumA));
                    fused = true;
                    m->last.bwd.t3b += 1;
                } else if (d3d_bwd_applies(m, ly, fuse, acc, hand)) {
                    ALQ_TRY(d3d_bwd_launch(ctx, ly.d3f, N, ly.dout.p, fz.in_bound, ly.din.p, ly.din.p + ly.din.delta, fz.osumB));
                    fused = true;
                    m->last.bwd.d3b = 1;
                } else
                ALQ_TRY(gemm_launch(ctx, ly.bwd, ly.dout, ly.din, nullptr, 0, acc, N, PROF_IGEMM_BWD, fuse, &fused));
                if (hand) {
                    unsigned *dst = mine == m->amax_a ? m->amax_b : m->amax_a;
                    ALQ_TRY(k_rowmax_u32(ctx, m->amax_tiles, ly.bwd.p4.a.tpg * 4, N, dst));
                    prev->dout_amax = dst;
                }
            }
        }
        if (prev_param && fused) prev->delta_ready = true;
    }
    return ALQ_OK;
}

static int run_backward_general(alq_model *m, int N, const DropSpec *drop, bool layer_sums = false) {
    alq_ctx *ctx = m->ctx;
    const int nl = (int)m->layers.size();
    m->last.lsum = layer_sums ? 1 : 0;
    m->last.bwd = {};
    for (int i = nl - 1; i >= 0; --i) {
        Layer &ly = m->layers[i];
        const bool isfc = ly.spec.type == ALQ_FC;
        const bool prev_is_src = (i > 0 && m->layers[i - 1].out_is_skip_src && ly.spec.skip_src < 0);
        if (drop && drop->on(i))
            ALQ_TRY(k_dropout(ctx, isfc ? flat_view(ly.dout) : ly.dout, N, drop->first_sample, drop->seed, i, drop->keep_prob));
        if (ly.spec.type == ALQ_POOL) {
            if (i == 0) break;
            bool fused = false;
            ALQ_TRY(k_pool_bwd(ctx, ly.dout, ly.din, ly.argmax, ly.spec.k, ly.lo, N, prev_is_src ? 1 : 0, nullptr, nullptr, &fused, 1));
            continue;
        }
        View dv = isfc ? flat_view(ly.dout) : ly.dout;
        View av = isfc ? flat_view(ly.out) : ly.out;
        if (layer_sums)
            ALQ_TRY(k_lsum_sweep(ctx, dv, ly.spec.relu ? &av : nullptr, isfc, ly.ls_field, N,
                                 m->ls_part + (size_t)ly.pidx * m->max_batch * m->ls_nslab_max, m->ls_nslab_max));
        else
            ALQ_TRY(k_mask_chansum(ctx, dv, ly.spec.relu ? &av : nullptr, ly.dsum, N));
        if (ly.pidx == 0) break;
        const int acc = prev_is_src ? 1 : 0;
        if (isfc) {
            ALQ_REQUIRE(!acc, ALQ_EUNSUPPORTED, "layer %d: fc consumer of a skip source", i);
            if (ly.dense_fc_small) {
                bool fused = false;
                ALQ_TRY(k_fc_small_bwd(ctx, ly.dout.p, ly.spec.cout, ly.d_Wp, ly.F, N, ly.din.p, nullptr, nullptr, 0, &fused));
            } else {
                ALQ_TRY(gemm_launch(ctx, ly.bwd, ly.dout, flat_view(ly.din), nullptr, 0, 0, N, PROF_IGEMM_BWD, nullptr, nullptr, 0.f));
            }
        } else {
            ALQ_TRY(gemm_launch(ctx, ly.bwd, ly.dout, ly.din, nullptr, 0, acc, N, PROF_IGEMM_BWD));
        }
    }
    return ALQ_OK;
}

static int run_param_grads(alq_model *m, const float *d_x, int N, int sum_n, float *d_out, long long P) {
    alq_ctx *ctx = m->ctx;
    long long need = 0;
    for (Layer &ly : m->layers) {
        if (ly.pidx < 0 || ly.spec.type == ALQ_FC) continue;
        const bool convt = ly.spec.type == ALQ_CONVT;
        need = std::max(need, wgrad_partial_floats(convt ? ly.in : ly.dout, convt ? ly.dout : ly.in, ly.spec.k) * N);
    }
    if ((size_t)need > m->wg_partial_len) {
        ALQ_TRY(m->dalloc(&m->wg_partial, (size_t)need));
        m->wg_partial_len = (size_t)need;
    }
    long long off = 0;
    const long long stride = sum_n ? 0 : P;
    for (size_t i = 0; i < m->layers.size(); ++i) {
        Layer &ly = m->layers[i];
        if (ly.pidx < 0) continue;
        View in = ly.in;
        if (i == 0) in.p = const_cast<float *>(d_x);
        const int one[3] = {1, 1, 1};
        if (ly.spec.type == ALQ_CONV) {
            ALQ_TRY(k_wgrad(ctx, ly.dout, in, ly.spec.k, one, ly.lo, N, sum_n, m->wg_partial, d_out + off, stride));
            ALQ_TRY(k_bgrad(ctx, ly.dout, N, sum_n, d_out + off + ly.w_elems, stride));
        } else if (ly.spec.type == ALQ_CONVT) {
            ALQ_TRY(k_wgrad(ctx, in, ly.dout, ly.spec.k, ly.spec.s, ly.lo, N, sum_n, m->wg_partial, d_out + off, stride));
            ALQ_TRY(k_bgrad(ctx, ly.dout, N, sum_n, d_out + off + ly.w_elems, stride));
        } else {
            ALQ_TRY(k_fc_wgrad(ctx, ly.dout.p, in, ly.spec.cout, N, sum_n, d_out + off, stride));
            ALQ_TRY(k_bgrad(ctx, flat_view(ly.dout), N, sum_n, d_out + off + ly.w_elems, stride));
        }
        off += ly.w_elems + ly.b_elems;
    }
    ALQ_REQUIRE(off == P, ALQ_EINVAL, "parameter count mismatch");
    return ALQ_OK;
}

static int run_grad_sqnorms(alq_model *m, const float *d_x, int N, double *d_sq) {
    alq_ctx *ctx = m->ctx;
    const int one[3] = {1, 1, 1};
    long long need = 0;
    for (Layer &ly : m->layers) {
        if (ly.pidx < 0 || ly.spec.type == ALQ_FC) continue;
        const bool convt = ly.spec.type == ALQ_CONVT;
        need = std::max(need, gnorm_partials(convt ? ly.in : ly.dout, convt ? ly.dout : ly.in, ly.spec.k, convt ? ly.spec.s : one,
                                             ly.lo) * N);
    }
    if ((size_t)need > m->gn_partial_len) {
        ALQ_TRY(m->dalloc(&m->gn_partial, (size_t)need));
        m->gn_partial_len = (size_t)need;
    }
    const int ld = 2 * m->L;
    for (size_t i = 0; i < m->layers.size(); ++i) {
        Layer &ly = m->layers[i];
        if (ly.pidx < 0) continue;
        View in = ly.in;
        if (i == 0) in.p = const_cast<float *>(d_x);
        const int col = 2 * ly.pidx;
        if (ly.spec.type == ALQ_CONV) {
            ALQ_TRY(k_gnorm_weight(ctx, ly.dout, in, ly.spec.k, one, ly.lo, N, m->gn_partial, d_sq, ld, col));
            ALQ_TRY(k_gnorm_bias(ctx, ly.dout, N, d_sq, ld, col + 1));
        } else if (ly.spec.type == ALQ_CONVT) {
            ALQ_TRY(k_gnorm_weight(ctx, in, ly.dout, ly.spec.k, ly.spec.s, ly.lo, N, m->gn_partial, d_sq, ld, col));
            ALQ_TRY(k_gnorm_bias(ctx, ly.dout, N, d_sq, ld, col + 1));
        } else {
            ALQ_TRY(k_gnorm_fc(ctx, ly.dout.p, ly.spec.cout, in, N, d_sq, ld, col));
        }
    }
    return ALQ_OK;
}

static int run_diag_fisher(alq_model *m, const float *d_x, int N, double *d_acc) {
    alq_ctx *ctx = m->ctx;
    const int one[3] = {1, 1, 1};
    if (!m->df_scratch) {
        long long need = 1;
        for (Layer &ly : m->layers) {
            if (ly.pidx < 0) continue;
            need = std::max(need, (long long)m->max_batch * ly.spec.cout);
            if (ly.spec.type == ALQ_FC) continue;
            const bool convt = ly.spec.type == ALQ_CONVT;
            need = std::max(need, dfisher_weight_scratch(convt ? ly.in : ly.dout, convt ? ly.dout : ly.in, ly.spec.k,
                                                         convt ? ly.spec.s : one, ly.lo, m->max_batch));
        }
        ALQ_TRY(m->dalloc(&m->df_scratch, (size_t)need));
    }
    long long off = 0;
    for (size_t i = 0; i < m->layers.size(); ++i) {
        Layer &ly = m->layers[i];
        if (ly.pidx < 0) continue;
        View in = ly.in;
        if (i == 0) in.p = const_cast<float *>(d_x);
        double *aw = d_acc + off, *ab = aw + ly.w_elems;
        if (ly.spec.type == ALQ_CONV) {
            ALQ_TRY(k_dfisher_weight(ctx, ly.dout, in, ly.spec.k, one, ly.lo, N, m->df_scratch, aw));
            ALQ_TRY(k_dfisher_bias(ctx, ly.dout, N, m->df_scratch, ab));
        } else if (ly.spec.type == ALQ_CONVT) {
            ALQ_TRY(k_dfisher_weight(ctx, in, ly.dout, ly.spec.k, ly.spec.s, ly.lo, N, m->df_scratch, aw));
            ALQ_TRY(k_dfisher_bias(ctx, ly.dout, N, m->df_scratch, ab));
        } else {
            ALQ_TRY(k_dfisher_fc(ctx, ly.dout.p, ly.spec.cout, in, N, m->df_scratch, aw, ab));
        }
        off += ly.w_elems + ly.b_elems;
    }
    ALQ_REQUIRE(off == alq_model_num_params(m), ALQ_EINVAL, "parameter count mismatch");
    return ALQ_OK;
}

static int make_drop(const alq_model *m, float keep_prob, uint64_t seed, int64_t first_sample, const int32_t *h_layers, int n_layers,
                     DropSpec *d) {
// ... 671 lines not shown
    } guard(m->ctx);
    ALQ_TRY(prepare_call(m, true));
    ALQ_TRY(run_forward(m, d_x, N, true));
    ALQ_TRY(k_softmax(m->ctx, m->logits, m->nclass, N, m->post, nullptr));
    ALQ_TRY(run_backward(m, d_x, N));
    int nblocks = 0;
    ALQ_TRY(k_fisher_finalize(m->ctx, m->Spart, m->nslab, m->nslab_max, m->max_batch, m->S, m->L, m->sizes, m->post,
                              d_p1_in, N, diag_load, d_p1_out, d_g0, d_g1, d_A, d_trace, m->Apart, &nblocks));
    if (d_Asum) ALQ_TRY(k_reduce_Asum(m->ctx, m->Apart, nblocks, m->L * m->L, d_Asum));
    return ALQ_OK;
}

static int stage_rows(alq_model *m, const float *d_pool, const int64_t *d_rows, int N) {
    ALQ_REQUIRE(d_pool && d_rows, ALQ_EINVAL, "null pool / row list");
    if (!m->x_stage) ALQ_TRY(m->dalloc(&m->x_stage, (size_t)m->max_batch * m->epp));
    return gather_rows_impl(m->ctx, d_pool, d_rows, N, m->epp, m->x_stage);
}

int alq_forward_rows(alq_model *m, const float *d_pool, const int64_t *d_rows, int N, float *d_post, int64_t *d_pred,
                     float *d_feat, int feature_layer_idx) {
    ALQ_REQUIRE(m != nullptr, ALQ_EINVAL, "alq_forward_rows: null model");
    ALQ_REQUIRE(N >= 0 && N <= m->max_batch, ALQ_EINVAL, "alq_forward_rows: N=%d exceeds max_batch=%d", N, m->max_batch);
    if (N == 0) return ALQ_OK;
    ALQ_HIP(hipSetDevice(m->ctx->device));
    ALQ_TRY(stage_rows(m, d_pool, d_rows, N));
    return alq_forward(m, m->x_stage, N, d_post, d_pred, d_feat, feature_layer_idx);
}

int alq_fisher_rows(alq_model *m, const float *d_pool, const int64_t *d_rows, int N, const float *d_p1_in, double diag_load,
                    float *d_p1_out, double *d_g0, double *d_g1, double *d_A, double *d_trace, double *d_Asum) {
    ALQ_REQUIRE(m != nullptr, ALQ_EINVAL, "alq_fisher_rows: null model");
    ALQ_REQUIRE(N >= 0 && N <= m->max_batch, ALQ_EINVAL, "alq_fisher_rows: N=%d exceeds max_batch=%d", N, m->max_batch);
    ALQ_HIP(hipSetDevice(m->ctx->device));
    if (N > 0) ALQ_TRY(stage_rows(m, d_pool, d_rows, N));
    return alq_fisher(m, N > 0 ? m->x_stage : d_pool, N, d_p1_in, diag_load, d_p1_out, d_g0, d_g1, d_A, d_trace, d_Asum);
}

int alq_topk_merge(const double *h_keys, const int64_t *h_idx, int64_t n, int64_t B, int64_t *h_out_idx,
                   int64_t *n_out) {
    ALQ_REQUIRE(n >= 0 && B >= 0 && (n == 0 || (h_keys && h_idx)) && (B == 0 || h_out_idx) && n_out, ALQ_EINVAL,
                "alq_topk_merge: bad argument");
    std::vector<std::pair<uint64_t, int64_t>> v;
    v.reserve((size_t)n);
    for (int64_t i = 0; i < n; ++i)
        if (h_idx[i] >= 0) {
            double k = h_keys[i] == 0.0 ? 0.0 : h_keys[i];
            uint64_t b;
            std::memcpy(&b, &k, sizeof(b));
            v.emplace_back(b, h_idx[i]);
        }
    std::sort(v.begin(), v.end());
    const int64_t m = std::min<int64_t>(B, (int64_t)v.size());
    for (int64_t i = 0; i < m; ++i) h_out_idx[i] = v[(size_t)i].second;
    *n_out = m;
    return ALQ_OK;
}

static const char *kProfNames[PROF_NUM] = {"igemm_fwd", "igemm_bwd", "elementwise", "reduce", "fc_small",
                                           "igemm3_fwd", "igemm3_bwd", "direct_conv", "igemm_f16x2", "gnorm",
                                           "committee", "eval"};

int alq_prof_enable(alq_ctx *ctx, int on) {
    ALQ_REQUIRE(ctx != nullptr, ALQ_EINVAL, "null ctx");
    ctx->prof_on = on != 0;
    ctx->prof_every = on > 1 ? on : 1;
    ctx->prof_pass = 0;
    return ALQ_OK;
}

int alq_prof_reset(alq_ctx *ctx) {
    ALQ_REQUIRE(ctx != nullptr, ALQ_EINVAL, "null ctx");
    ALQ_TRY(ctx->prof_collect());
    for (int c = 0; c < PROF_NUM; ++c) {
        ctx->prof[c].ms = 0; ctx->prof[c].launches = 0; ctx->prof[c].flops = 0;
    }
    return ALQ_OK;
}

int alq_prof_num_classes(void) { return PROF_NUM; }
const char *alq_prof_class_name(int cls) { return (cls >= 0 && cls < PROF_NUM) ? kProfNames[cls] : ""; }

int alq_prof_read(alq_ctx *ctx, int cls, double *ms, int64_t *launches, double *flops) {
    ALQ_REQUIRE(ctx && cls >= 0 && cls < PROF_NUM, ALQ_EINVAL, "alq_prof_read: bad class");
    ALQ_TRY(ctx->prof_collect());
    if (ms) *ms = ctx->prof[cls].ms;
    if (launches) *launches = ctx->prof[cls].launches;
    if (flops) *flops = ctx->prof[cls].flops;
    return ALQ_OK;
}

int alq_model_debug_copy(alq_model *m, int layer_idx, int what, int N, float *d_out, int64_t *elems_out) {
    ALQ_REQUIRE(m && d_out && N >= 1 && N <= m->max_batch, ALQ_EINVAL, "alq_model_debug_copy: bad argument");
    ALQ_HIP(hipSetDevice(m->ctx->device));
    if (what == 4) {
        if (elems_out) *elems_out = (int64_t)N * m->L;
        return debug_f64_copy(m->ctx, m->S, (long long)N * m->L, d_out);
    }
    if (what == 5) {
        const Layer &head = m->layers.back();
        ALQ_REQUIRE(head.fc_part2 && m->last.fwd.head_fused, ALQ_EUNSUPPORTED, "the last pass did not run the fused fc head");
        const int ns = m->last.fwd.c3 ? 4 : head.fc_slices2;
        if (elems_out) *elems_out = (int64_t)N * ns;
        ALQ_HIP(hipMemcpyAsync(d_out, m->last.fwd.c3 ? head.c3_part : head.fc_part2, (size_t)N * ns * sizeof(float), hipMemcpyDeviceToDevice,
                               m->ctx->stream));
        return ALQ_OK;
    }
    ALQ_REQUIRE(layer_idx >= 0 && layer_idx < (int)m->layers.size(), ALQ_EINVAL, "bad layer index");
    const Layer &ly = m->layers[layer_idx];
    if (what >= 6 && what <= 10) {
        ALQ_REQUIRE(ly.spec.type == ALQ_FC && ly.fwd.size() == 1 && ly.fwd[0].pfc.ok && ly.weights_set, ALQ_EUNSUPPORTED, "layer %d has no streaming-GEMM weights", layer_idx);
        if (what == 10) {
            int32_t wd[4] = {ly.fwd[0].pfc.w_exp, ly.bwd.pfc.w_exp, 0, 0};
            std::memcpy(&wd[2], &ly.bwd_l1, 8);
            if (elems_out) *elems_out = 4;
            ALQ_HIP(hipMemcpyAsync(d_out, wd, 16, hipMemcpyHostToDevice, m->ctx->stream));
            ALQ_HIP(hipStreamSynchronize(m->ctx->stream));
            return ALQ_OK;
        }
        const FcGemmPlan &pl = what <= 7 ? ly.fwd[0].pfc : ly.bwd.pfc;
        const void *src = (what & 1) ? pl.d_W16 : pl.d_W;
        ALQ_REQUIRE(pl.ok && src, ALQ_EUNSUPPORTED, "layer %d: this form is not packed", layer_idx);
        const int64_t e = (int64_t)pl.K * pl.N * ((what & 1) ? 2 : 3) / 2;
        if (elems_out) *elems_out = e;
        ALQ_HIP(hipMemcpyAsync(d_out, src, (size_t)e * 4, hipMemcpyDeviceToDevice, m->ctx->stream));
        return ALQ_OK;
    }
    if (what >= 11 && what <= 13) {
        if (what == 11) {
            ALQ_REQUIRE(ly.osum && m->last.call_fisher, ALQ_EUNSUPPORTED, "layer %d: no channel sums of its output in the last pass", layer_idx);
            if (elems_out) *elems_out = (int64_t)N * ly.out.vox();
            ALQ_HIP(hipMemcpyAsync(d_out, ly.osum, (size_t)N * ly.out.vox() * sizeof(float), hipMemcpyDeviceToDevice, m->ctx->stream));
            return ALQ_OK;
        }
        if (what == 12) {
            const View &v = ly.out;
            ALQ_REQUIRE(v.sg && ly.signs_ready && ((v.C | v.cs | v.c0) & 3) == 0 && ((int64_t)N * v.vox() * v.cs) % 16 == 0, ALQ_EUNSUPPORTED,
                        "layer %d: no sign field of its output in the last pass", layer_idx);
            if (elems_out) *elems_out = (int64_t)N * v.vox() * v.cs / 16;
            ALQ_HIP(hipMemcpyAsync(d_out, v.sg, (size_t)N * v.vox() * v.cs / 4, hipMemcpyDeviceToDevice, m->ctx->stream));
            return ALQ_OK;
        }
        ALQ_REQUIRE(ly.spec.type == ALQ_POOL && ly.argmax && ((int64_t)N * ly.out.vox() * ly.out.C) % 4 == 0, ALQ_EUNSUPPORTED, "layer %d has no arg-max field", layer_idx);
        if (elems_out) *elems_out = (int64_t)N * ly.out.vox() * ly.out.C / 4;
        ALQ_HIP(hipMemcpyAsync(d_out, ly.argmax, (size_t)N * ly.out.vox() * ly.out.C, hipMemcpyDeviceToDevice, m->ctx->stream));
        return ALQ_OK;
    }
    if (what == 0 || what == 1) {
        const Layer &head = m->layers.back();
        ALQ_REQUIRE(!(layer_idx + 2 == (int)m->layers.size() && head.spec.type == ALQ_FC &&
                      (what == 0 ? m->last.fwd.head_fused
                                 : (m->last.call_fisher && head.fc_maskbits != nullptr && two_slot_allowed()))),
                    ALQ_EUNSUPPORTED, "layer %d: this tensor is not materialised in a Fisher pass (fc head fused into the layer: "
                    "create the model under ALQ_NO_FC_BITS=1 to keep it)", layer_idx);
        const View &v = what == 0 ? ly.out : ly.dout;
        if (elems_out) *elems_out = (int64_t)N * v.elems();
        return debug_view_copy(m->ctx, v, N, d_out);
    }
    ALQ_REQUIRE(ly.pidx >= 0 && (what == 2 || what == 3), ALQ_EINVAL, "layer has no channel-sum fields");
    const bool isfc = ly.spec.type == ALQ_FC;
    const int64_t e = (int64_t)N * (isfc ? 1 : (what == 2 ? ly.in.vox() : ly.out.vox()));
    if (elems_out) *elems_out = e;
    ALQ_HIP(hipMemcpyAsync(d_out, what == 2 ? ly.asum : ly.dsum, e * sizeof(float), hipMemcpyDeviceToDevice,
                           m->ctx->stream));
    return ALQ_OK;
}

int alq_model_engine_info(alq_model *m, int what) {
    ALQ_REQUIRE(m, ALQ_EINVAL, "alq_model_engine_info: bad argument");
    switch (what) {
        case ALQ_INFO_SUBNORMALS_OK:
            ALQ_HIP(hipSetDevice(m->ctx->device));
            return c3d_subnormals_ok(m->ctx);
        case ALQ_INFO_C3D_FWD: return m->last.fwd.c3 ? 1 : 0;
        case ALQ_INFO_C3D_BWD: return m->last.bwd.c3_bwd ? 1 : 0;
        case ALQ_INFO_C3D_ONE_ACC:
            for (const Layer &ly : m->layers)
                if (ly.c3f.ok) return ly.c3f.oneacc;
            return 0;
        case ALQ_INFO_FLIP_OVERFLOW: {
            ALQ_HIP(hipSetDevice(m->ctx->device));
            if (!m->flip_overflow) return 0;
            unsigned h = 0;
            ALQ_HIP(hipMemcpyAsync(&h, m->flip_overflow, sizeof(unsigned), hipMemcpyDeviceToHost, m->ctx->stream));
            ALQ_HIP(hipStreamSynchronize(m->ctx->stream));
            return h > 0x7fffffffu ? 0x7fffffff : (int)h;
        }
        case ALQ_INFO_F16_DERIVED: return m->last.fwd.f16_derived ? 1 : 0;
        case ALQ_INFO_T3D_FWD: return m->last.fwd.t3f;
        case ALQ_INFO_T3D_BWD: return m->last.bwd.t3b;
        case ALQ_INFO_E3D_BWD: return m->last.bwd.e3b;
        case ALQ_INFO_D3D_FWD: return m->last.fwd.d3f;
        case ALQ_INFO_D3D_BWD: return m->last.bwd.d3b;
        case ALQ_INFO_F3D_FWD: return m->last.fwd.f3f;
        case ALQ_INFO_C3D_BWD_FORM: return m->last.bwd.c3_bwd ? m->sw.c3_bwd_rows : 0;
        case ALQ_INFO_HOST_PACK_ELEMS: return m->host_pack_elems > 0x7fffffffll ? 0x7fffffff : (int)m->host_pack_elems;
        case ALQ_INFO_LSUM: return m->last.lsum;
        case ALQ_INFO_DCP_FORM: return m->last.fwd.dcp;
        case ALQ_INFO_E3D_BWD_FORM: return m->last.bwd.e3b_form;
        default: break;
    }
    set_error("alq_model_engine_info: bad argument");
    return ALQ_EINVAL;
}

int alq_debug_set(int key, int value) {
    ALQ_REQUIRE(key >= 0 && key < ALQ_NKNOBS, ALQ_EINVAL, "alq_debug_set: bad key");
    g_knob_override[key] = value > 0 ? value : -1;
    g_dbg_knobs[key] = value;
    return ALQ_OK;
}

int alq_debug_set_stamp_buffer(void *d_buf) {
    g_igemm2_dbg = reinterpret_cast<unsigned long long *>(d_buf);
    return ALQ_OK;
}

int alq_synth_patches(alq_ctx *ctx, uint64_t seed, int64_t first_id, int64_t n, int64_t epp, float *d_out) {
    ALQ_REQUIRE(ctx && (n == 0 || d_out), ALQ_EINVAL, "alq_synth_patches: null argument");
    if (n == 0) return ALQ_OK;
    ALQ_HIP(hipSetDevice(ctx->device));
    return synth_impl(ctx, seed, first_id, n, epp, d_out);
}

}
```

### nn-active-learning_amd/csrc/model_types.h

```cpp
#pragma once
#include <algorithm>

#include "alq_internal.h"

namespace alq {

struct Layer {
    alq_layer_t spec;
    int pidx = -1;
    View in, out;
    View din, dout;
    int lo[3] = {0, 0, 0};
    bool dense_fc_small = false;
    int64_t F = 0;
    int64_t w_elems = 0, b_elems = 0;
    float *d_bias = nullptr;
    float *d_Wp = nullptr;
    std::vector<Gemm> fwd;
    std::vector<Gemm> fwd_co;
    int fwd_co_w = 0;
    Igemm4Plan fwd_all;
    Gemm bwd;
    bool has_bwd = false;
    bool weights_set = false;
    float *d_Wres = nullptr;
    bool fallback_stale = false;
    uint8_t *argmax = nullptr;
    float *asum = nullptr, *dsum = nullptr;
    double *ls_field = nullptr;
    float *osum = nullptr;
    bool delta_ready = false;
    bool signs_ready = false;
    bool dsum_partial = false;
    float *fc_partials = nullptr;
    unsigned *fc_maskbits = nullptr;
    float *fc_wv = nullptr;
    unsigned *fc_wv16 = nullptr;
    float fc_wv_amax = 0.f;
    const unsigned *dout_amax = nullptr;
    unsigned *amax_fwd = nullptr;
    float dout_vec_amax = 0.f;
    double bwd_l1 = 0;
    float dout_bound = 0.f;
    float *d_W32 = nullptr;
    float fwd_l1 = 0.f;
    float out_l1 = 0.f, out_bmax = 0.f;
    unsigned *bound_fwd = nullptr;
    float *fc_part2 = nullptr;
    int fc_slices2 = 0;
    C3dPlan c3f, c3b;
    D3dPlan d3f;
    F3dPlan f3f;
    E3dPlan e3b;
    T3dPlan t3f, t3b;
    float *c3_part = nullptr, *c3_asum = nullptr;
    unsigned short *fc_wv16c = nullptr;
    const unsigned short *dout_vec16c = nullptr;
    const unsigned *dout_bits = nullptr;
    const float *dout_vec = nullptr;
    const unsigned *dout_vec16 = nullptr;
    int fc_slices = 0;
    bool out_is_skip_src = false;
    std::vector<std::vector<int>> class_taps;
    std::vector<float> hv_hW;
    int hv_src = 0;
    bool hv_stale = false;
    float *hv_W = nullptr;
    double *hv_A = nullptr, *hv_D = nullptr, *hv_Ra = nullptr, *hv_Rd = nullptr;
};

}

struct PassInfo {
    struct Fwd {
        bool head_fused = false;
        bool c3 = false;
        int t3f = 0;
        int d3f = 0;
        int f3f = 0;
        int dcp = 0;
        bool f16_derived = false;
    } fwd;
    struct Bwd {
        bool c3_bwd = false;
        int t3b = 0;
        int e3b = 0;
        int e3b_form = 0;
        int d3b = 0;
    } bwd;
    int lsum = 0;
    bool call_fisher = false;
};

struct alq_model {
    alq_ctx *ctx = nullptr;
    int max_batch = 0;
    alq::EngineSwitches sw;
    PassInfo last;
    unsigned *amax_a = nullptr, *amax_b = nullptr, *amax_tiles = nullptr;
    unsigned *flip_cnt = nullptr, *flip_list = nullptr;
    int flip_cap = 0;
    unsigned *bound_all = nullptr;
    unsigned *in_amax = nullptr;
    bool v3_fwd_f16 = false;
    unsigned *flip_overflow = nullptr;
    size_t amax_tiles_len = 0;
    int in_dims[4] = {1, 1, 1, 1};
    int nclass = 0;
    int L = 0;
    std::vector<alq::Layer> layers;
    std::vector<void *> allocs;
    float *logits = nullptr, *dlogits = nullptr, *post = nullptr;
    double *S = nullptr, *sizes = nullptr, *Apart = nullptr;
    double *Spart = nullptr;
    int *nslab = nullptr;
    int nslab_max = 1;
    float *wg_partial = nullptr;
    size_t wg_partial_len = 0;
    double *gn_partial = nullptr;
    size_t gn_partial_len = 0;
    double *df_scratch = nullptr;
    double *ls_part = nullptr;
    std::vector<int> ls_nslab;
    int ls_nslab_max = 0;
    float *x_stage = nullptr;
    int64_t epp = 0;
    int f16_fwd_derived = 0;
    int64_t host_pack_elems = 0;
    void *d_wscal = nullptr;
    bool hv_ready = false;
    double *hv_part = nullptr;
    double *hv_p64 = nullptr;

    template <typename T>
    int dalloc(T **p, size_t count) {
        void *q = nullptr;
        const size_t bytes = std::max<size_t>(count * sizeof(T), 256);
        if (hipMalloc(&q, bytes) != hipSuccess) {
            alq::set_error("hipMalloc of %zu bytes failed", bytes);
            return ALQ_ENOMEM;
        }
        allocs.push_back(q);
        *p = reinterpret_cast<T *>(q);
        return ALQ_OK;
    }
};

template <typename T, typename D>
int ensure(alq_model *m, D **d, size_t count) {
    T *p = static_cast<T *>(*d);
    if (!p) ALQ_TRY(m->dalloc(&p, count));
    *d = p;
    return ALQ_OK;
}

template <typename T, typename D>
int upload(alq_model *m, D **d, const std::vector<T> &h) {
    ALQ_TRY(ensure<T>(m, d, h.size()));
    ALQ_HIP(hipMemcpyAsync(*d, h.data(), h.size() * sizeof(T), hipMemcpyHostToDevice, m->ctx->stream));
    return ALQ_OK;
}

template <typename T, typename D>
int upload_release(alq_model *m, D **d, std::vector<T> *h) {
    ALQ_TRY(upload(m, d, *h));
    ALQ_HIP(hipStreamSynchronize(m->ctx->stream));
    std::vector<T>().swap(*h);
    return ALQ_OK;
}

namespace alq { int refresh_fallback_forms(alq_model *m); }
```

Measured before the change: 285,100.

## Fuse transposed-conv upsample backward into following d3d conv backward kernel

```diff
diff --git a/include/alq.h b/include/alq.h
--- a/include/alq.h
+++ b/include/alq.h
@@ -234,7 +234,8 @@
     ALQ_INFO_HOST_PACK_ELEMS = 14,
     ALQ_INFO_LSUM = 15,
     ALQ_INFO_DCP_FORM = 16,
-    ALQ_INFO_E3D_BWD_FORM = 17
+    ALQ_INFO_E3D_BWD_FORM = 17,
+    ALQ_INFO_UP2_BWD_FORM = 19
 };
 int alq_model_engine_info(alq_model *m, int what);
 
diff --git a/nn-active-learning_amd/csrc/alq_internal.h b/nn-active-learning_amd/csrc/alq_internal.h
--- a/nn-active-learning_amd/csrc/alq_internal.h
+++ b/nn-active-learning_amd/csrc/alq_internal.h
@@ -420,9 +420,12 @@
     void *d_Whi = nullptr, *d_Wlo = nullptr;
     std::vector<unsigned short> h_Bhi, h_Blo;
     void *d_Bhi = nullptr, *d_Blo = nullptr;
+    bool no_up2_fuse = false;
 };
 void d3d_bwd_pack(D3dPlan *plan, const float *W);
 int d3d_bwd_launch(alq_ctx *ctx, const D3dPlan &plan, int N, const float *dout, float in_bound, float *dinA, float *dinB, float *sumB);
+int d3d_bwd_up2_launch(alq_ctx *ctx, const D3dPlan &plan, const T3dPlan &up2, int N, const float *up, float up_bound, const unsigned char *mask_bits,
+                       float *dsum, float in_bound, float *dinA, float *dinB, float *sumB);
 int d3d_build(const View &in, const View &out, const int k[3], const int lo[3], const int s[3], D3dPlan *plan);
 void d3d_pack(D3dPlan *plan, const float *W );
 int d3d_fwd_launch(alq_ctx *ctx, const D3dPlan &plan, int N, const float *inA, const float *inB, const unsigned *amaxA, const unsigned *amaxB,
diff --git a/nn-active-learning_amd/csrc/d3d.hip b/nn-active-learning_amd/csrc/d3d.hip
--- a/nn-active-learning_amd/csrc/d3d.hip
+++ b/nn-active-learning_amd/csrc/d3d.hip
@@ -5,6 +5,7 @@
 #include <cmath>
 #include <cstdlib>
 #include <cstring>
+#include <utility>
 #include <vector>
 
 namespace alq {
@@ -412,8 +413,291 @@
     }
 }
 
+struct D3UArgs {
+    const float *up;
+    const unsigned short *UW;
+    const unsigned char *mask_bits;
+    float *dsum;
+    const unsigned short *Whi, *Wlo;
+    float *dinA, *dinB;
+    float *sumB;
+    float u_scale, u_inv;
+    float scale, scale11, inv;
+    int N;
+};
+constexpr int DU_ROWB = 36 * 16;
+constexpr int DU_SET = 6 * 2 * DU_ROWB;
+constexpr int DU_WAVE = 2 * DU_SET;
+constexpr int DU_WOFF = DB_STRIP;
+constexpr int DU_WBYTES = 18 * 1024;
+constexpr int DU_SOFF = DU_WOFF + DU_WBYTES;
+constexpr int DU_LDS = DU_SOFF + 4 * DU_WAVE;
+constexpr int DU_UNITS = 3 + 4 * 16;
+constexpr int DU_FIRST[11] = {0, 3, 8, 16, 25, 33, 42, 50, 59, 64, 67};
+constexpr int du_kind(int u) { return u < 3 ? 0 : ((u - 3) % 16 < 6 ? 0 : ((u - 3) % 16 < 15 ? 1 : 2)); }
+constexpr int du_tile(int u) { return u < 3 ? 0 : (u - 3) / 16; }
+constexpr int du_pos(int u) { return u < 3 ? u : 3 + 6 * ((u - 3) / 16) + (u - 3) % 16; }
+constexpr int du_mfmas(int r) {
+    int n = 0;
+    for (int u = DU_FIRST[r]; u < DU_FIRST[r + 1]; ++u) n += du_kind(u) == 1 ? 3 : 0;
+    return n;
+}
+template <int U0, typename F, int... I>
+__device__ __forceinline__ void du_run(F &f, std::integer_sequence<int, I...>) { (f(IC<U0 + I>{}), ...); }
+
+__global__ __launch_bounds__(256) __attribute__((amdgpu_waves_per_eu(1, 1))) void d3d_bwd_up2_kernel(const D3UArgs a) {
+    extern __shared__ __attribute__((aligned(16))) char d3lds[];
+    const int lane = threadIdx.x & 63, wave = __builtin_amdgcn_readfirstlane((int)(threadIdx.x >> 6));
+    const int cb = wave & 1, rg = wave >> 1;
+    char *strip = d3lds;
+    char *const ustrip = d3lds + DU_SOFF + wave * DU_WAVE;
+    for (int i = threadIdx.x; i < DB_STRIP / 16; i += 256) reinterpret_cast<i32x4 *>(strip)[i] = i32x4{0, 0, 0, 0};
+    for (int i = threadIdx.x; i < DU_WBYTES / 16; i += 256)
+        reinterpret_cast<i32x4 *>(d3lds + DU_WOFF)[i] = reinterpret_cast<const i32x4 *>(a.UW)[i];
+    if (lane < 48)
+        *reinterpret_cast<i32x4 *>(ustrip + (lane >> 1) * DU_ROWB + (34 + (lane & 1)) * 16) = i32x4{0, 0, 0, 0};
+    __syncthreads();
+    const int n = lane & 15, kg = lane >> 4;
+    f16x8 wh[15], wl[15];
+#pragma unroll
+    for (int c = 0; c < 15; ++c) {
+        wh[c] = *reinterpret_cast<const f16x8 *>(a.Whi + ((size_t)(cb * 15 + c) * 64 + lane) * 8);
+        wl[c] = *reinterpret_cast<const f16x8 *>(a.Wlo + ((size_t)(cb * 15 + c) * 64 + lane) * 8);
+    }
+#pragma unroll
+    for (int c = 0; c < 15; ++c) asm volatile("" : "+a"(wh[c]), "+a"(wl[c]));
+
+    const __amdgpu_buffer_rsrc_t up_rsrc = sw_rsrc(a.up, (unsigned long long)a.N * 32 * 32 * 32 * 8 * 4);
+    const __amdgpu_buffer_rsrc_t m_rsrc = sw_rsrc(a.mask_bits, (unsigned long long)a.N * 4096 * 4);
+    const __amdgpu_buffer_rsrc_t ds_rsrc = sw_rsrc(a.dsum, (unsigned long long)a.N * 4096 * 4);
+    const __amdgpu_buffer_rsrc_t o_rsrc = sw_rsrc(cb ? a.dinB : a.dinA, (unsigned long long)a.N * 4096 * 64);
+    const __amdgpu_buffer_rsrc_t u_rsrc = sw_rsrc(a.sumB, a.sumB ? (unsigned long long)a.N * 4096 * 4 : 0ull);
+
+    const unsigned ldU = (unsigned)lane * 16u;
+    const int w_offU = ((lane >> 1) + (lane >> 5)) * 16 + (lane & 1) * 8;
+    const char *const fU = ustrip + ((2 * n + kg) + ((2 * n + kg) >> 4)) * 16;
+    const char *const uwl = d3lds + DU_WOFF + lane * 16;
+    const unsigned mk_off = (unsigned)n * 4u + (unsigned)kg;
+    const unsigned sm_off = kg < 2 ? (unsigned)n * 4u + (unsigned)kg * 64u : SW_OOB;
+    char *const iw_base = strip + (4 * wave + 4) * DB_SLOT + (kg >> 1) * DB_KG + (n + 1) * 16 + (kg & 1) * 8;
+    const char *const f01 = strip + 8 * rg * DB_SLOT + (kg & 1) * DB_KG + (n + (kg >> 1)) * 16;
+    const char *const f22 = strip + 8 * rg * DB_SLOT + (kg >> 1) * DB_SLOT + (kg & 1) * DB_KG + (n + 2) * 16;
+    const unsigned e_out = (unsigned)n * 64u + (unsigned)kg * 16u;
+    const unsigned e_sum = (kg == 0 && cb == 1) ? (unsigned)n * 4u : SW_OOB;
+
+    const int G = (int)gridDim.x, b0 = (int)blockIdx.x;
+    const int npw = a.N > b0 ? (a.N - b0 + G - 1) / G : 0;
+    auto patch_of = [&](int i) __attribute__((always_inline)) { return b0 + (i < npw ? i : npw - 1) * G; };
+
+    struct DuT { int p, iz, p2, iz2, img; bool v, v2; };
+    f32x4 UR[9];
+    unsigned MK[4];
+    f32x4 uc = f32x4{0.f, 0.f, 0.f, 0.f};
+    float s_odd = 0.f;
+    const float usc = a.u_scale;
+    auto uload = [&](auto POS, int p, int iz, bool v) __attribute__((always_inline)) {
+        constexpr int pos = decltype(POS)::value;
+        constexpr int tz = pos < 3 ? pos : ((pos - 3) % 6) >> 1;
+        constexpr int yo = pos < 3 ? 8 : 6 - 2 * ((pos - 3) / 6) + ((pos - 3) % 6 & 1);
+        bool ok = v;
+        if (tz == 2) ok = ok && iz < 15;
+        if (pos < 3) ok = ok && wave < 3;
+        const int so = sw_s((((unsigned)p * 32u + (unsigned)(2 * iz + tz)) * 32u + (unsigned)(8 * wave + yo)) * 1024u);
+        UR[pos % 9] = __builtin_bit_cast(f32x4, __builtin_amdgcn_raw_buffer_load_b128(up_rsrc, (int)(ok ? ldU : SW_OOB), so, 0));
+    };
+    auto umask = [&](auto K, int p, int iz, bool v) __attribute__((always_inline)) {
+        constexpr int k = decltype(K)::value;
+        const int so = sw_s((((unsigned)p * 16u + (unsigned)iz) * 16u + (unsigned)(4 * wave + 3 - k)) * 64u);
+        MK[k] = (unsigned)(unsigned char)__builtin_amdgcn_raw_buffer_load_b8(m_rsrc, (int)(v ? mk_off : SW_OOB), so, 0);
+    };
+    f16x8 GFh[2], GFl[2], GW0[2], GW1[2];
+    auto gread = [&](auto K, auto GG) __attribute__((always_inline)) {
+        constexpr int k = decltype(K)::value, g = decltype(GG)::value, tz = g / 3, ty = g % 3;
+        constexpr int set = ty == 2 ? ((k & 1) ^ 1) : (k & 1), slot = ty == 2 ? 2 * tz : 2 * tz + ty;
+        const char *fp = fU + set * DU_SET + 2 * slot * DU_ROWB;
+        GFh[g & 1] = *reinterpret_cast<const f16x8 *>(fp);
+        GFl[g & 1] = *reinterpret_cast<const f16x8 *>(fp + DU_ROWB);
+        GW0[g & 1] = *reinterpret_cast<const f16x8 *>(uwl + (2 * g) * 1024);
+        GW1[g & 1] = *reinterpret_cast<const f16x8 *>(uwl + (2 * g + 1) * 1024);
+    };
+    auto unit = [&](auto UU, const DuT &t) __attribute__((always_inline)) {
+        constexpr int u = decltype(UU)::value, kind = du_kind(u), k = du_tile(u);
+        if constexpr (kind == 0) {
+            constexpr int pos = du_pos(u);
+            constexpr int set = pos < 3 ? 1 : (k & 1), slot = pos < 3 ? 2 * pos : (pos - 3) % 6;
+            char *dst = ustrip + set * DU_SET + 2 * slot * DU_ROWB + w_offU;
+            const f32x4 R = UR[pos % 9];
+            const float x0 = R.x * usc, x1 = R.y * usc, x2 = R.z * usc, x3 = R.w * usc;
+            const f16x2 h01 = __builtin_convertvector(f32x2{x0, x1}, f16x2), h23 = __builtin_convertvector(f32x2{x2, x3}, f16x2);
+            const f16x2 l01 = __builtin_convertvector(f32x2{x0 - (float)h01.x, x1 - (float)h01.y}, f16x2);
+            const f16x2 l23 = __builtin_convertvector(f32x2{x2 - (float)h23.x, x3 - (float)h23.y}, f16x2);
+            *reinterpret_cast<i32x2 *>(dst) = i32x2{__builtin_bit_cast(int, h01), __builtin_bit_cast(int, h23)};
+            *reinterpret_cast<i32x2 *>(dst + DU_ROWB) = i32x2{__builtin_bit_cast(int, l01), __builtin_bit_cast(int, l23)};
+            if constexpr (pos + 9 < 27) uload(IC<(pos + 9) % 27>{}, t.p, t.iz, t.v);
+            else uload(IC<(pos + 9) % 27>{}, t.p2, t.iz2, t.v2);
+            if constexpr (pos >= 3 && (pos - 3) % 6 == 5) gread(IC<k>{}, IC<0>{});
+        } else if constexpr (kind == 1) {
+            constexpr int g = (u - 3) % 16 - 6;
+            if constexpr (g < 8) gread(IC<k>{}, IC<g + 1>{});
+            const f16x8 fh = GFh[g & 1], fl = GFl[g & 1], w0 = GW0[g & 1], w1 = GW1[g & 1];
+            f32x4 c = g == 0 ? f32x4{0.f, 0.f, 0.f, 0.f} : uc;
+            c = __builtin_amdgcn_mfma_f32_16x16x32_f16(w1, fh, c, 0, 0, 0);
+            c = __builtin_amdgcn_mfma_f32_16x16x32_f16(w0, fl, c, 0, 0, 0);
+            c = __builtin_amdgcn_mfma_f32_16x16x32_f16(w0, fh, c, 0, 0, 0);
+            uc = c;
+        } else {
+            const unsigned crow = ((unsigned)t.p * 16u + (unsigned)t.iz) * 16u + (unsigned)(4 * wave + 3 - k);
+            const unsigned nb = MK[k];
+            f32x4 v = f32x4{uc.x * a.u_inv, uc.y * a.u_inv, uc.z * a.u_inv, uc.w * a.u_inv};
+            v.x = (nb & 1u) ? v.x : 0.f; v.y = (nb & 2u) ? v.y : 0.f;
+            v.z = (nb & 4u) ? v.z : 0.f; v.w = (nb & 8u) ? v.w : 0.f;
+            umask(IC<k>{}, t.p2, t.iz2, t.v2);
+            float s = (v.x + v.y) + (v.z + v.w);
+            s += __shfl_xor(s, 16, 64);
+            s += __shfl_xor(s, 32, 64);
+            if constexpr ((k & 1) == 0) s_odd = s;
+            else
+                __builtin_amdgcn_raw_buffer_store_b32(__builtin_bit_cast(int, kg == 1 ? s_odd : s), ds_rsrc, (int)(t.v ? sm_off : SW_OOB), sw_s(crow * 64u), 0);
+            const float sc = t.v ? a.scale : 0.f, sc11 = t.v ? a.scale11 : 0.f;
+            char *dst = iw_base + t.img * DB_PLANE - k * DB_SLOT;
+            const f16x2 h01 = __builtin_convertvector(f32x2{v.x * sc, v.y * sc}, f16x2), h23 = __builtin_convertvector(f32x2{v.z * sc, v.w * sc}, f16x2);
+            const f16x2 l01 = __builtin_convertvector(f32x2{__builtin_fmaf((float)h01.x, -2048.f, v.x * sc11), __builtin_fmaf((float)h01.y, -2048.f, v.y * sc11)}, f16x2);
+            const f16x2 l23 = __builtin_convertvector(f32x2{__builtin_fmaf((float)h23.x, -2048.f, v.z * sc11), __builtin_fmaf((float)h23.y, -2048.f, v.w * sc11)}, f16x2);
+            *reinterpret_cast<i32x2 *>(dst) = i32x2{__builtin_bit_cast(int, h01), __builtin_bit_cast(int, h23)};
+            *reinterpret_cast<i32x2 *>(dst + DB_ROWB) = i32x2{__builtin_bit_cast(int, l01), __builtin_bit_cast(int, l23)};
+        }
+    };
+    auto plane_of = [&](int q, int img) __attribute__((always_inline)) {
+        DuT t;
+        t.p = patch_of(q >> 4); t.iz = q & 15; t.v = (q >> 4) < npw;
+        t.p2 = patch_of((q + 1) >> 4); t.iz2 = (q + 1) & 15; t.v2 = ((q + 1) >> 4) < npw;
+        t.img = img;
+        return t;
+    };
+
+    f32x4 acc[3][8], acx[3][8];
+#pragma unroll
+    for (int st = 0; st < 3; ++st)
+#pragma unroll
+        for (int ry = 0; ry < 8; ++ry) { acc[st][ry] = f32x4{0.f, 0.f, 0.f, 0.f}; acx[st][ry] = f32x4{0.f, 0.f, 0.f, 0.f}; }
+    f32x4 okeep[2];
+    okeep[0] = okeep[1] = f32x4{0.f, 0.f, 0.f, 0.f};
+
+    auto epi_row = [&](auto ST, auto RY, int p, int zo, bool tv) __attribute__((always_inline)) {
+        constexpr int st = decltype(ST)::value, ry = decltype(RY)::value;
+        const unsigned vrow = (unsigned)sw_s((((unsigned)p * 16u + (unsigned)(tv ? zo : 0)) * 16u + (unsigned)(8 * rg + ry)) * 16u);
+        const f32x4 c = acc[st][ry], cx = acx[st][ry];
+        if (!D3_START) { acc[st][ry] = f32x4{0.f, 0.f, 0.f, 0.f}; acx[st][ry] = f32x4{0.f, 0.f, 0.f, 0.f}; }
+        const float v0 = __builtin_fmaf(cx.x, 0x1p-11f, c.x) * a.inv, v1 = __builtin_fmaf(cx.y, 0x1p-11f, c.y) * a.inv;
+        const float v2 = __builtin_fmaf(cx.z, 0x1p-11f, c.z) * a.inv, v3 = __builtin_fmaf(cx.w, 0x1p-11f, c.w) * a.inv;
+        const f32x4 o = f32x4{v0, v1, v2, v3};
+        okeep[ry & 1] = o;
+        __builtin_amdgcn_raw_buffer_store_b128(__builtin_bit_cast(i32x4, o), o_rsrc, (int)(tv ? e_out : SW_OOB), (int)(vrow * 64u), 0);
+        ALQ_STORE_HOLD("v"(o));
+        float s_ = (v0 + v1) + (v2 + v3);
+        s_ += __shfl_xor(s_, 16, 64);
+        s_ += __shfl_xor(s_, 32, 64);
+        __builtin_amdgcn_raw_buffer_store_b32(__builtin_bit_cast(int, s_), u_rsrc, (int)(tv ? e_sum : SW_OOB), (int)(vrow * 4u), 0);
+    };
+
+    auto step = [&](auto JJ, int i, int s) __attribute__((always_inline)) {
+        constexpr int J = decltype(JJ)::value;
+        constexpr int S0 = (J + 1) % 3, S1 = J, S2 = (J + 2) % 3;
+        __builtin_amdgcn_sched_barrier(0);
+        const int q = 16 * i + s;
+        const int p = patch_of(i);
+        const int img = q & 1;
+        const DuT t = plane_of(q + 1, img ^ 1);
+        asm volatile("s_waitcnt lgkmcnt(0)\n\ts_barrier" ::: "memory");
+        const char *fa = f01 + img * DB_PLANE, *fb = f22 + img * DB_PLANE;
+        f16x8 Fh[2][2], Fl[2][2];
+        auto frag = [&](auto R, f16x8 *fh, f16x8 *fl) __attribute__((always_inline)) {
+            constexpr int r = decltype(R)::value;
+            fh[0] = *reinterpret_cast<const f16x8 *>(fa + r * DB_SLOT);
+            fl[0] = *reinterpret_cast<const f16x8 *>(fa + r * DB_SLOT + DB_ROWB);
+            fh[1] = *reinterpret_cast<const f16x8 *>(fb + r * DB_SLOT);
+            fl[1] = *reinterpret_cast<const f16x8 *>(fb + r * DB_SLOT + DB_ROWB);
+        };
+        frag(IC<0>{}, Fh[0], Fl[0]);
+        auto mm = [&](auto ST, auto RY, auto KS, const f16x8 &xh, const f16x8 &xl) __attribute__((always_inline)) {
+            constexpr int st = decltype(ST)::value, ry = decltype(RY)::value, ks = decltype(KS)::value;
+            constexpr bool first = D3_START && ks == 0;
+            const f32x4 zero = f32x4{0.f, 0.f, 0.f, 0.f};
+            acx[st][ry] = __builtin_amdgcn_mfma_f32_16x16x32_f16(wl[ks], xh, first ? zero : acx[st][ry], 0, 0, 0);
+            acc[st][ry] = __builtin_amdgcn_mfma_f32_16x16x32_f16(wh[ks], xh, first ? zero : acc[st][ry], 0, 0, 0);
+            acx[st][ry] = __builtin_amdgcn_mfma_f32_16x16x32_f16(wh[ks], xl, acx[st][ry], 0, 0, 0);
+        };
+        auto unit_t = [&](auto UU) __attribute__((always_inline)) { unit(UU, t); };
+        auto block = [&](auto R) __attribute__((always_inline)) {
+            constexpr int r = decltype(R)::value;
+            __builtin_amdgcn_sched_barrier(0);
+            if constexpr (r + 1 < 10) frag(IC<r + 1>{}, Fh[(r + 1) % 2], Fl[(r + 1) % 2]);
+            if constexpr (r == 0) epi_row(IC<S0>{}, IC<7>{}, p, s - 2, s >= 2);
+            if constexpr (r >= 3) epi_row(IC<S2>{}, IC<r - 3>{}, p, s - 1, s >= 1);
+            const f16x8 ph = Fh[r % 2][0], pl = Fl[r % 2][0], qh = Fh[r % 2][1], ql = Fl[r % 2][1];
+            constexpr int nu = DU_FIRST[r + 1] - DU_FIRST[r];
+            auto slot = [&](auto SL) __attribute__((always_inline)) {
+                constexpr int sl = decltype(SL)::value, pi = sl / 3, dz = sl % 3;
+                auto at_slot = [&](auto JC) __attribute__((always_inline)) {
+                    constexpr int j = decltype(JC)::value;
+                    if constexpr ((15 * j) / nu == sl) unit_t(IC<DU_FIRST[r] + j>{});
+                };
+                du_run<0>(at_slot, std::make_integer_sequence<int, nu>{});
+                constexpr bool act = pi == 0 ? r <= 7 : (pi == 1 ? (r >= 1 && r <= 8) : (pi == 2 ? r >= 2 : (pi == 3 ? r <= 7 : r >= 2)));
+                constexpr int ry = (pi == 0 || pi == 3) ? r : (pi == 1 ? r - 1 : r - 2);
+                constexpr int st = dz == 0 ? S0 : (dz == 1 ? S1 : S2);
+                if constexpr (act) mm(IC<st>{}, IC<(act ? ry : 0)>{}, IC<dz * 5 + pi>{}, pi < 3 ? ph : qh, pi < 3 ? pl : ql);
+            };
+            du_run<0>(slot, std::make_integer_sequence<int, 15>{});
+#pragma unroll
+            for (int m = 0; m < 9 * ((r == 0 || r == 9) ? 2 : ((r == 1 || r == 8) ? 3 : 5)) + du_mfmas(r); ++m) {
+                __builtin_amdgcn_sched_group_barrier(0x008, 1, 0);
+                __builtin_amdgcn_sched_group_barrier(SW_FILL_MASK, D3_PIPE, 0);
+            }
+        };
+        block(IC<0>{}); block(IC<1>{}); block(IC<2>{}); block(IC<3>{}); block(IC<4>{});
+        block(IC<5>{}); block(IC<6>{}); block(IC<7>{}); block(IC<8>{}); block(IC<9>{});
+        __builtin_amdgcn_sched_barrier(0);
+        const f32x4 k0 = okeep[0], k1 = okeep[1];
+        asm volatile("" :: "v"(k0), "v"(k1));
+    };
+
+    if (npw > 0) {
+        {
+            const DuT t = plane_of(0, 0);
+            uload(IC<0>{}, t.p, 0, true); uload(IC<1>{}, t.p, 0, true); uload(IC<2>{}, t.p, 0, true);
+            uload(IC<3>{}, t.p, 0, true); uload(IC<4>{}, t.p, 0, true); uload(IC<5>{}, t.p, 0, true);
+            uload(IC<6>{}, t.p, 0, true); uload(IC<7>{}, t.p, 0, true); uload(IC<8>{}, t.p, 0, true);
+            umask(IC<0>{}, t.p, 0, true); umask(IC<1>{}, t.p, 0, true); umask(IC<2>{}, t.p, 0, true); umask(IC<3>{}, t.p, 0, true);
+            auto unit_t = [&](auto UU) __attribute__((always_inline)) { unit(UU, t); };
+            du_run<0>(unit_t, std::make_integer_sequence<int, DU_UNITS>{});
+            __builtin_amdgcn_sched_barrier(0);
+        }
+        for (int i = 0; i < npw; ++i) {
+            for (int k = 0; k < 5; ++k) {
+                step(IC<0>{}, i, 3 * k);
+                step(IC<1>{}, i, 3 * k + 1);
+                step(IC<2>{}, i, 3 * k + 2);
+            }
+            step(IC<0>{}, i, 15);
+            __builtin_amdgcn_sched_barrier(0);
+            const int p = patch_of(i);
+            epi_row(IC<2>{}, IC<7>{}, p, 14, true);
+            epi_row(IC<0>{}, IC<0>{}, p, 15, true); epi_row(IC<0>{}, IC<1>{}, p, 15, true);
+            epi_row(IC<0>{}, IC<2>{}, p, 15, true); epi_row(IC<0>{}, IC<3>{}, p, 15, true);
+            epi_row(IC<0>{}, IC<4>{}, p, 15, true); epi_row(IC<0>{}, IC<5>{}, p, 15, true);
+            epi_row(IC<0>{}, IC<6>{}, p, 15, true); epi_row(IC<0>{}, IC<7>{}, p, 15, true);
+#pragma unroll
+            for (int ry = 0; ry < 8; ++ry) { acc[0][ry] = f32x4{0.f, 0.f, 0.f, 0.f}; acx[0][ry] = f32x4{0.f, 0.f, 0.f, 0.f}; }
+            __builtin_amdgcn_sched_barrier(0);
+            asm volatile("s_nop 7" :: "v"(okeep[0]), "v"(okeep[1]) : "memory");
+        }
+    }
+}
+
 int d3d_build(const View &in, const View &out, const int k[3], const int lo[3], const int s[3], D3dPlan *plan) {
     plan->ok = false;
+    plan->no_up2_fuse = getenv("ALQ_NO_UP2_BWD_FUSE") != nullptr;
     if (getenv("ALQ_NO_D3D")) return ALQ_OK;
     if (!is_conv3_same(k, lo, s)) return ALQ_OK;
     if (!(in.D == 16 && in.H == 16 && in.W == 16 && out.D == 16 && out.H == 16 && out.W == 16 && in.C == 32 && in.split == 16 && in.cs == 16 && in.c0 == 0 &&
@@ -473,6 +757,26 @@
     return sweep_launch(ctx, d3d_bwd_kernel, sweep_grid(ctx, N, 1), 256, DB_STRIP, a);
 }
 
+int d3d_bwd_up2_launch(alq_ctx *ctx, const D3dPlan &plan, const T3dPlan &up2, int N, const float *up, float up_bound, const unsigned char *mask_bits,
+                       float *dsum, float in_bound, float *dinA, float *dinB, float *sumB) {
+    ALQ_REQUIRE(plan.ok && plan.d_Bhi && plan.d_Blo && up2.ok && up2.kind == 0 && up2.d_W, ALQ_EINVAL, "d3d: backward weights not set");
+    ALQ_REQUIRE(up && mask_bits && dsum && dinA && dinB && in_bound > 0.f && up_bound > 0.f, ALQ_EINVAL, "d3d: missing argument");
+    SWEEP_REQUIRE_PATCHES(N, "d3d");
+    if (N <= 0) return ALQ_OK;
+    const int e_in = f16_pair_exp(&in_bound, 1), e_up = f16_pair_exp(&up_bound, 1);
+    D3UArgs a;
+    a.up = up; a.UW = reinterpret_cast<const unsigned short *>(up2.d_W); a.mask_bits = mask_bits; a.dsum = dsum;
+    a.Whi = reinterpret_cast<const unsigned short *>(plan.d_Bhi); a.Wlo = reinterpret_cast<const unsigned short *>(plan.d_Blo);
+    a.dinA = dinA; a.dinB = dinB; a.sumB = sumB;
+    a.u_scale = std::ldexp(1.f, e_up); a.u_inv = std::ldexp(1.f, -(e_up + up2.w_exp));
+    a.scale = std::ldexp(1.f, e_in); a.scale11 = std::ldexp(1.f, e_in + 11); a.inv = std::ldexp(1.f, -(e_in + plan.w_exp)); a.N = N;
+    unsigned g = sweep_grid(ctx, N, 1);
+    if (g_dbg_knobs[KNOB_E3D_GRID_CAP] > 0) g = std::min<unsigned>(g, (unsigned)g_dbg_knobs[KNOB_E3D_GRID_CAP]);
+    ProfScope ps(ctx, PROF_IGEMM_F16, (plan.flops_per_patch + up2.flops_per_patch) * N);
+    if (ps.active) ctx->prof[PROF_IGEMM_F16].launches += 1;
+    return sweep_launch(ctx, d3d_bwd_up2_kernel, g, 256, DU_LDS, a);
+}
+
 int d3d_fwd_launch(alq_ctx *ctx, const D3dPlan &plan, int N, const float *inA, const float *inB, const unsigned *amaxA, const unsigned *amaxB,
                    const float *bias, int relu, float *out, unsigned char *sg, float *osum) {
     ALQ_REQUIRE(plan.ok && plan.d_Whi && plan.d_Wlo, ALQ_EINVAL, "d3d: weights not set");
diff --git a/nn-active-learning_amd/csrc/engine_switches.h b/nn-active-learning_amd/csrc/engine_switches.h
--- a/nn-active-learning_amd/csrc/engine_switches.h
+++ b/nn-active-learning_amd/csrc/engine_switches.h
@@ -16,11 +16,12 @@
     KNOB_NO_CONV_POOL = 7,
     KNOB_DCP_NARROW = 8,
     KNOB_E3D_GRID_CAP = 9,
-    ALQ_NKNOBS = 10
+    KNOB_NO_UP2_BWD_FUSE = 10,
+    ALQ_NKNOBS = 11
 };
 
 struct EngineSwitches {
-    int knobs[ALQ_NKNOBS] = {0, 0, 0, 0, 0, 0, 0, 0, 0, 0};
+    int knobs[ALQ_NKNOBS] = {0, 0, 0, 0, 0, 0, 0, 0, 0, 0, 0};
     int disable_v2 = 0;
     int disable_v3 = 0;
     int disable_v4 = 0;
diff --git a/nn-active-learning_amd/csrc/igemm2.hip b/nn-active-learning_amd/csrc/igemm2.hip
--- a/nn-active-learning_amd/csrc/igemm2.hip
+++ b/nn-active-learning_amd/csrc/igemm2.hip
@@ -507,7 +507,7 @@
 int g_no_f16x2 = 0;
 int g_no_xcd_order = 0;
 int g_no_fixed = 0;
-int g_dbg_knobs[ALQ_NKNOBS] = {0, 0, 0, 0, 0, 0, 0, 0, 0, 0};
+int g_dbg_knobs[ALQ_NKNOBS] = {0, 0, 0, 0, 0, 0, 0, 0, 0, 0, 0};
 
 template <int NTW, bool WRES, int GEO, bool SUMS>
 static int launch2_s(alq_ctx *ctx, const Igemm2Plan &plan, const Igemm2Args &a, unsigned grid) {
diff --git a/nn-active-learning_amd/csrc/model.hip b/nn-active-learning_amd/csrc/model.hip
--- a/nn-active-learning_amd/csrc/model.hip
+++ b/nn-active-learning_amd/csrc/model.hip
@@ -75,7 +75,7 @@
     return ALQ_OK;
 }
 
-static int g_knob_override[ALQ_NKNOBS] = {-1, -1, -1, -1, -1, -1, -1, -1, -1, -1};
+static int g_knob_override[ALQ_NKNOBS] = {-1, -1, -1, -1, -1, -1, -1, -1, -1, -1, -1};
 
 static void apply_knobs(const alq_model *m) {
     for (int k = 0; k < ALQ_NKNOBS; ++k) g_dbg_knobs[k] = g_knob_override[k] >= 0 ? g_knob_override[k] : m->sw.knobs[k];
@@ -970,6 +970,12 @@
            !ly.dout.split && ly.dout.cs == 16 && ly.dout.c0 == 0 && ly.din.split == 16 && ly.din.cs == 16 && ly.din.c0 == 0 && ly.din.C == 32;
 }
 
+static bool up2_bwd_fuse_candidate(const alq_model *m, const Layer &ly, const Layer &prev, const Igemm2Fuse &fz) {
+    return !g_dbg_knobs[KNOB_NO_UP2_BWD_FUSE] && !prev.d3f.no_up2_fuse && ly.t3b.kind == 0 && fz.mask && fz.mask_bits && prev.spec.type == ALQ_CONV &&
+           prev.d3f.ok && prev.d3f.d_Bhi && !m->sw.no_d3d && !m->sw.no_d3b && prev.pidx > 0 && !prev.out_is_skip_src && !prev.dout_bits &&
+           ly.din.p == prev.dout.p && !prev.dout.split && prev.dout.cs == 16 && prev.dout.c0 == 0 && ly.dout.C == 8 && ly.dout.cs == 8 && ly.dout.c0 == 0;
+}
+
 static int run_backward_main(alq_model *m, const float *d_x, int N);
 static int run_backward(alq_model *m, const float *d_x, int N) {
     const int rc = run_backward_main(m, d_x, N);
@@ -1000,9 +1006,40 @@
         }
     }
     int e3_conv = -1;
+    struct { int layer = -1; float bound = 0.f; const unsigned char *mask_bits = nullptr; float *dsum = nullptr; } held;
+    auto launch_held = [&]() -> int {
+        if (held.layer < 0) return ALQ_OK;
+        Layer &up = m->layers[held.layer];
+        held.layer = -1;
+        return t3d_bwd_launch(ctx, up.t3b, up.dout, up.din, N, held.bound, held.mask_bits, held.dsum);
+    };
+    auto box_sums = [&](int bi) -> int {
+        const Layer &bl = m->layers[bi];
+        const bool bfc = bl.spec.type == ALQ_FC;
+        const float *as1 = bl.asum, *as2 = nullptr;
+        if (!bfc) {
+            if (bi == 0) as1 = bl.in.C == 1 ? d_x : bl.asum;
+            else as1 = m->layers[bi - 1].osum;
+            if (bl.spec.skip_src >= 0) as2 = m->layers[bl.spec.skip_src].osum;
+        }
+        double *Sdst = m->Spart + (size_t)bl.pidx * m->max_batch * m->nslab_max;
+        SideStream beside(ctx);
+        if (bl.spec.type == ALQ_CONVT) {
+            ALQ_TRY(k_boxdot_convT(ctx, bl.dsum, as1, as2, bl.in.D, bl.in.H, bl.in.W, bl.spec.k, bl.spec.s, bl.lo, N, Sdst, m->nslab_max));
+        } else if (bfc) {
+            const int one[3] = {1, 1, 1}, zero[3] = {0, 0, 0};
+            ALQ_TRY(k_boxdot_conv(ctx, bl.dsum, bl.asum, nullptr, 1, 1, 1, one, zero, N, Sdst, m->nslab_max));
+        } else {
+            ALQ_TRY(k_boxdot_conv(ctx, bl.dsum, as1, as2, bl.out.D, bl.out.H, bl.out.W, bl.spec.k, bl.lo, N, Sdst, m->nslab_max));
+        }
+        return ALQ_OK;
+    };
+    int late_sums = -1;
     for (int i = nl - 1; i >= 0; --i) {
         Layer &ly = m->layers[i];
         const bool prev_is_src = (i > 0 && m->layers[i - 1].out_is_skip_src && ly.spec.skip_src < 0);
+        if (held.layer >= 0 && i != held.layer - 1) ALQ_TRY(launch_held());
+        if (late_sums >= 0 && i < late_sums - 1) { ALQ_TRY(box_sums(late_sums)); late_sums = -1; }
         if (e3d_bwd_applies(m, i, prev_is_src)) {
             Layer &cv = m->layers[i - 1], &p1 = m->layers[i - 2], &c0 = m->layers[i - 3];
             ALQ_TRY(e3d_bwd_launch(ctx, cv.e3b, N, cv.dout.p, ly.dout.p, ly.argmax, cv.out.sg, p1.argmax, p1.out.sg, cv.dsum, c0.dsum, cv.dout_bound, m->sw.e3d_rows != 0));
@@ -1037,24 +1074,9 @@
             View av = isfc ? flat_view(ly.out) : ly.out;
             ALQ_TRY(k_mask_chansum(ctx, dv, ly.spec.relu ? &av : nullptr, ly.dsum, N));
         }
-        const float *as1 = ly.asum, *as2 = nullptr;
-        if (!isfc) {
-            if (i == 0) as1 = ly.in.C == 1 ? d_x : ly.asum;
-            else as1 = m->layers[i - 1].osum;
-            if (ly.spec.skip_src >= 0) as2 = m->layers[ly.spec.skip_src].osum;
-        }
-        double *Sdst = m->Spart + (size_t)ly.pidx * m->max_batch * m->nslab_max;
-        {
-            SideStream beside(ctx);
-            if (ly.spec.type == ALQ_CONVT) {
-                ALQ_TRY(k_boxdot_convT(ctx, ly.dsum, as1, as2, ly.in.D, ly.in.H, ly.in.W, ly.spec.k, ly.spec.s, ly.lo, N, Sdst, m->nslab_max));
-            } else if (isfc) {
-                const int one[3] = {1, 1, 1}, zero[3] = {0, 0, 0};
-                ALQ_TRY(k_boxdot_conv(ctx, ly.dsum, ly.asum, nullptr, 1, 1, 1, one, zero, N, Sdst, m->nslab_max));
-            } else {
-                ALQ_TRY(k_boxdot_conv(ctx, ly.dsum, as1, as2, ly.out.D, ly.out.H, ly.out.W, ly.spec.k, ly.lo, N, Sdst, m->nslab_max));
-            }
-        }
+        if (held.layer >= 0 && (ly.pidx == 0 || i == e3_conv || isfc || ly.dout_bits)) ALQ_TRY(launch_held());
+        if (held.layer >= 0) late_sums = i;
+        else ALQ_TRY(box_sums(i));
         if (ly.pidx == 0) break;
         if (i == e3_conv) continue;
         const int acc = prev_is_src ? 1 : 0;
@@ -1153,15 +1175,31 @@
                 const unsigned *mine = ly.dout_amax;
                 ly.dout_amax = nullptr;
                 if (t3d_bwd_applies(m, ly, fuse, acc, hand, prev_param)) {
-                    ALQ_TRY(t3d_bwd_launch(ctx, ly.t3b, ly.dout, ly.din, N, fz.in_bound, fz.mask ? fz.mask_bits : nullptr, fz.osumA));
+                    if (up2_bwd_fuse_candidate(m, ly, *prev, fz)) {
+                        held.layer = i; held.bound = fz.in_bound; held.mask_bits = fz.mask_bits; held.dsum = fz.osumA;
+                    } else {
+                        ALQ_TRY(t3d_bwd_launch(ctx, ly.t3b, ly.dout, ly.din, N, fz.in_bound, fz.mask ? fz.mask_bits : nullptr, fz.osumA));
+                    }
                     fused = true;
                     m->last.bwd.t3b += 1;
                 } else if (d3d_bwd_applies(m, ly, fuse, acc, hand)) {
-                    ALQ_TRY(d3d_bwd_launch(ctx, ly.d3f, N, ly.dout.p, fz.in_bound, ly.din.p, ly.din.p + ly.din.delta, fz.osumB));
+                    if (held.layer >= 0) {
+                        const Layer &up = m->layers[held.layer];
+                        held.layer = -1;
+                        ALQ_TRY(d3d_bwd_up2_launch(ctx, ly.d3f, up.t3b, N, up.dout.p, held.bound, held.mask_bits, held.dsum, fz.in_bound, ly.din.p,
+                                                   ly.din.p + ly.din.delta, fz.osumB));
+                        m->last.bwd.up2_fused = 2;
+                        m->last.bwd.up2_layer = i + 1; m->last.bwd.up2_bound = held.bound; m->last.bwd.up2_mask = held.mask_bits;
+                    } else {
+                        ALQ_TRY(d3d_bwd_launch(ctx, ly.d3f, N, ly.dout.p, fz.in_bound, ly.din.p, ly.din.p + ly.din.delta, fz.osumB));
+                        if (m->last.bwd.t3b > 0) m->last.bwd.up2_fused = 1;
+                    }
                     fused = true;
                     m->last.bwd.d3b = 1;
-                } else
-                ALQ_TRY(gemm_launch(ctx, ly.bwd, ly.dout, ly.din, nullptr, 0, acc, N, PROF_IGEMM_BWD, fuse, &fused));
+                } else {
+                    ALQ_TRY(launch_held());
+                    ALQ_TRY(gemm_launch(ctx, ly.bwd, ly.dout, ly.din, nullptr, 0, acc, N, PROF_IGEMM_BWD, fuse, &fused));
+                }
                 if (hand) {
                     unsigned *dst = mine == m->amax_a ? m->amax_b : m->amax_a;
                     ALQ_TRY(k_rowmax_u32(ctx, m->amax_tiles, ly.bwd.p4.a.tpg * 4, N, dst));
@@ -1171,6 +1209,8 @@
         }
         if (prev_param && fused) prev->delta_ready = true;
     }
+    ALQ_TRY(launch_held());
+    if (late_sums >= 0) ALQ_TRY(box_sums(late_sums));
     return ALQ_OK;
 }
 
@@ -2148,6 +2188,10 @@
                                  : (m->last.call_fisher && head.fc_maskbits != nullptr && two_slot_allowed()))),
                     ALQ_EUNSUPPORTED, "layer %d: this tensor is not materialised in a Fisher pass (fc head fused into the layer: "
                     "create the model under ALQ_NO_FC_BITS=1 to keep it)", layer_idx);
+        if (what == 1 && m->last.call_fisher && m->last.bwd.up2_fused == 2 && layer_idx + 1 == m->last.bwd.up2_layer) {
+            const Layer &up = m->layers[m->last.bwd.up2_layer];
+            ALQ_TRY(t3d_bwd_launch(m->ctx, up.t3b, up.dout, up.din, N, m->last.bwd.up2_bound, m->last.bwd.up2_mask, nullptr));
+        }
         const View &v = what == 0 ? ly.out : ly.dout;
         if (elems_out) *elems_out = (int64_t)N * v.elems();
         return debug_view_copy(m->ctx, v, N, d_out);
@@ -2193,6 +2237,7 @@
         case ALQ_INFO_LSUM: return m->last.lsum;
         case ALQ_INFO_DCP_FORM: return m->last.fwd.dcp;
         case ALQ_INFO_E3D_BWD_FORM: return m->last.bwd.e3b_form;
+        case ALQ_INFO_UP2_BWD_FORM: return m->last.bwd.up2_fused;
         default: break;
     }
     set_error("alq_model_engine_info: bad argument");
diff --git a/nn-active-learning_amd/csrc/model_types.h b/nn-active-learning_amd/csrc/model_types.h
--- a/nn-active-learning_amd/csrc/model_types.h
+++ b/nn-active-learning_amd/csrc/model_types.h
@@ -87,6 +87,10 @@
         int e3b = 0;
         int e3b_form = 0;
         int d3b = 0;
+        int up2_fused = 0;
+        int up2_layer = -1;
+        float up2_bound = 0.f;
+        const unsigned char *up2_mask = nullptr;
     } bwd;
     int lsum = 0;
     bool call_fisher = false;
```

Result: no change. 287,700 (median of 6 runs) (+0.9%).
